# jayleicn/ClipBERT

Measured on NVIDIA H100. Metric: clips/sec fwd+bwd MSRVTT ret (ResNet50+BERT-base), higher is better.
Workload: dtype bf16

## Files before the change

### clipbert_b200/csrc/common.cuh

```cuda
#pragma once
#include <cuda.h>
#include <cuda_bf16.h>
#include <cuda_runtime.h>
#include <stdint.h>

#include "drop_cfg.h"

namespace cb {

#ifndef CB_SPIN_LIMIT
#define CB_SPIN_LIMIT (1u << 24)
#endif

__device__ __forceinline__ uint32_t smem_u32(const void* p) {
  return static_cast<uint32_t>(__cvta_generic_to_shared(p));
}

__device__ __forceinline__ void pdl_wait() { asm volatile("griddepcontrol.wait;" ::: "memory"); }
__device__ __forceinline__ void pdl_trigger() { asm volatile("griddepcontrol.launch_dependents;" ::: "memory"); }

__device__ __forceinline__ void mbar_init(uint64_t* bar, uint32_t count) {
  asm volatile("mbarrier.init.shared::cta.b64 [%0], %1;" ::"r"(smem_u32(bar)), "r"(count));
}
__device__ __forceinline__ void fence_mbar_init() {
  asm volatile("fence.mbarrier_init.release.cluster;" ::: "memory");
}
__device__ __forceinline__ void fence_proxy_async_smem() {
  asm volatile("fence.proxy.async.shared::cta;" ::: "memory");
}
__device__ __forceinline__ void mbar_expect_tx(uint64_t* bar, uint32_t bytes) {
  asm volatile("mbarrier.arrive.expect_tx.shared::cta.b64 _, [%0], %1;" ::"r"(smem_u32(bar)),
               "r"(bytes)
               : "memory");
}
__device__ __forceinline__ void mbar_arrive(uint64_t* bar) {
  asm volatile("mbarrier.arrive.shared::cta.b64 _, [%0];" ::"r"(smem_u32(bar)) : "memory");
}
__device__ __forceinline__ bool mbar_try_wait(uint64_t* bar, uint32_t parity) {
  uint32_t ok;
  asm volatile(
      "{\n\t.reg .pred p;\n\t"
      "mbarrier.try_wait.parity.shared::cta.b64 p, [%1], %2, %3;\n\t"
      "selp.u32 %0, 1, 0, p;\n\t}"
      : "=r"(ok)
      : "r"(smem_u32(bar)), "r"(parity), "r"(2000u)
      : "memory");
  return ok != 0;
}
__device__ __forceinline__ void mbar_wait(uint64_t* bar, uint32_t parity) {
  uint32_t spins = 0;
  while (!mbar_try_wait(bar, parity)) {
    if (++spins > CB_SPIN_LIMIT) __trap();
  }
}

__device__ __forceinline__ void tma_prefetch_desc(const CUtensorMap* map) {
  asm volatile("prefetch.tensormap [%0];" ::"l"(map) : "memory");
}
__device__ __forceinline__ void tma_load_2d(void* smem_dst, const CUtensorMap* map, uint64_t* bar,
                                            int c0, int c1) {
  asm volatile(
      "cp.async.bulk.tensor.2d.shared::cluster.global.mbarrier::complete_tx::bytes "
      "[%0], [%1, {%3, %4}], [%2];" ::"r"(smem_u32(smem_dst)),
      "l"(map), "r"(smem_u32(bar)), "r"(c0), "r"(c1)
      : "memory");
}

__device__ __forceinline__ void bulk_load_1d(uint32_t smem_dst, const void* gsrc, uint32_t bytes, uint64_t* bar) {
  asm volatile("cp.async.bulk.shared::cluster.global.mbarrier::complete_tx::bytes [%0], [%1], %2, [%3];" ::"r"(smem_dst), "l"(gsrc),
               "r"(bytes), "r"(smem_u32(bar))
               : "memory");
}

__device__ __forceinline__ void tma_load_2d_s32(uint32_t smem_dst, const CUtensorMap* map, uint64_t* bar, int c0, int c1) {
  asm volatile(
      "cp.async.bulk.tensor.2d.shared::cluster.global.mbarrier::complete_tx::bytes "
      "[%0], [%1, {%3, %4}], [%2];" ::"r"(smem_dst),
      "l"(map), "r"(smem_u32(bar)), "r"(c0), "r"(c1)
      : "memory");
}

__device__ __forceinline__ void tma_load_3d(void* smem_dst, const CUtensorMap* map, uint64_t* bar, int c0, int c1, int c2) {
  asm volatile(
      "cp.async.bulk.tensor.3d.shared::cluster.global.mbarrier::complete_tx::bytes "
      "[%0], [%1, {%3, %4, %5}], [%2];" ::"r"(smem_u32(smem_dst)),
      "l"(map), "r"(smem_u32(bar)), "r"(c0), "r"(c1), "r"(c2)
      : "memory");
}

__device__ __forceinline__ void tma_store_2d(const CUtensorMap* map, const void* smem_src, int c0, int c1) {
  asm volatile("cp.async.bulk.tensor.2d.global.shared::cta.bulk_group [%0, {%2, %3}], [%1];" ::"l"(map),
               "r"(smem_u32(smem_src)), "r"(c0), "r"(c1)
               : "memory");
}
__device__ __forceinline__ void tma_store_2d_s32(const CUtensorMap* map, uint32_t smem_src, int c0, int c1) {
  asm volatile("cp.async.bulk.tensor.2d.global.shared::cta.bulk_group [%0, {%2, %3}], [%1];" ::"l"(map), "r"(smem_src), "r"(c0), "r"(c1)
               : "memory");
}
__device__ __forceinline__ uint4 lds128(uint32_t saddr) {
  uint4 v;
  asm volatile("ld.shared.v4.u32 {%0, %1, %2, %3}, [%4];" : "=r"(v.x), "=r"(v.y), "=r"(v.z), "=r"(v.w) : "r"(saddr));
  return v;
}
__device__ __forceinline__ void sts128(uint32_t saddr, uint4 v) {
  asm volatile("st.shared.v4.u32 [%0], {%1, %2, %3, %4};" ::"r"(saddr), "r"(v.x), "r"(v.y), "r"(v.z), "r"(v.w) : "memory");
}
__device__ __forceinline__ void tma_store_commit() { asm volatile("cp.async.bulk.commit_group;" ::: "memory"); }
template <int N>
__device__ __forceinline__ void tma_store_wait_read() {
  asm volatile("cp.async.bulk.wait_group.read %0;" ::"n"(N) : "memory");
}
template <int N>
__device__ __forceinline__ void tma_store_wait_all() {
  asm volatile("cp.async.bulk.wait_group %0;" ::"n"(N) : "memory");
}
__device__ __forceinline__ void named_bar_sync(uint32_t id, uint32_t nthreads) {
  asm volatile("bar.sync %0, %1;" ::"r"(id), "r"(nthreads) : "memory");
}

__device__ __forceinline__ void wgmma_fence() { asm volatile("wgmma.fence.sync.aligned;" ::: "memory"); }
__device__ __forceinline__ void wgmma_commit() { asm volatile("wgmma.commit_group.sync.aligned;" ::: "memory"); }
template <int N>
__device__ __forceinline__ void wgmma_wait() {
  asm volatile("wgmma.wait_group.sync.aligned %0;" ::"n"(N) : "memory");
}
template <int R>
__device__ __forceinline__ void wgmma_fence_acc(float (&d)[R]) {
#pragma unroll
  for (int i = 0; i < R; ++i) asm volatile("" : "+f"(d[i])::"memory");
}

__device__ __forceinline__ uint64_t gmma_desc(uint32_t smem_addr, uint32_t lbo, uint32_t sbo) {
  uint64_t d = 0;
  d |= static_cast<uint64_t>((smem_addr & 0x3FFFFu) >> 4);
  d |= static_cast<uint64_t>((lbo >> 4) & 0x3FFFu) << 16;
  d |= static_cast<uint64_t>((sbo >> 4) & 0x3FFFu) << 32;
  d |= 1ull << 62;
  return d;
}

template <int TA, int TB>
__device__ __forceinline__ void wgmma_bf16_n64(float (&d)[32], uint64_t adesc, uint64_t bdesc, uint32_t accumulate) {
  asm volatile(
      "{\n\t.reg .pred p;\n\t"
      "setp.ne.b32 p, %34, 0;\n\t"
      "wgmma.mma_async.sync.aligned.m64n64k16.f32.bf16.bf16 "
      "{"
      "%0, %1, %2, %3, %4, %5, %6, %7, %8, %9, %10, %11, %12, %13, %14, %15, "
      "%16, %17, %18, %19, %20, %21, %22, %23, %24, %25, %26, %27, %28, %29, %30, %31"
      "}, %32, %33, p, 1, 1, %35, %36;\n\t}"
      : "+f"(d[0]), "+f"(d[1]), "+f"(d[2]), "+f"(d[3]), "+f"(d[4]), "+f"(d[5]), "+f"(d[6]), "+f"(d[7]),
        "+f"(d[8]), "+f"(d[9]), "+f"(d[10]), "+f"(d[11]), "+f"(d[12]), "+f"(d[13]), "+f"(d[14]), "+f"(d[15]),
        "+f"(d[16]), "+f"(d[17]), "+f"(d[18]), "+f"(d[19]), "+f"(d[20]), "+f"(d[21]), "+f"(d[22]), "+f"(d[23]),
        "+f"(d[24]), "+f"(d[25]), "+f"(d[26]), "+f"(d[27]), "+f"(d[28]), "+f"(d[29]), "+f"(d[30]), "+f"(d[31])
      : "l"(adesc), "l"(bdesc), "r"(accumulate), "n"(TA), "n"(TB));
}
template <int TA, int TB>
__device__ __forceinline__ void wgmma_bf16_n128(float (&d)[64], uint64_t adesc, uint64_t bdesc, uint32_t accumulate) {
  asm volatile(
      "{\n\t.reg .pred p;\n\t"
      "setp.ne.b32 p, %66, 0;\n\t"
      "wgmma.mma_async.sync.aligned.m64n128k16.f32.bf16.bf16 "
      "{"
      "%0, %1, %2, %3, %4, %5, %6, %7, %8, %9, %10, %11, %12, %13, %14, %15, "
      "%16, %17, %18, %19, %20, %21, %22, %23, %24, %25, %26, %27, %28, %29, %30, %31, "
      "%32, %33, %34, %35, %36, %37, %38, %39, %40, %41, %42, %43, %44, %45, %46, %47, "
      "%48, %49, %50, %51, %52, %53, %54, %55, %56, %57, %58, %59, %60, %61, %62, %63"
      "}, %64, %65, p, 1, 1, %67, %68;\n\t}"
      : "+f"(d[0]), "+f"(d[1]), "+f"(d[2]), "+f"(d[3]), "+f"(d[4]), "+f"(d[5]), "+f"(d[6]), "+f"(d[7]),
        "+f"(d[8]), "+f"(d[9]), "+f"(d[10]), "+f"(d[11]), "+f"(d[12]), "+f"(d[13]), "+f"(d[14]), "+f"(d[15]),
        "+f"(d[16]), "+f"(d[17]), "+f"(d[18]), "+f"(d[19]), "+f"(d[20]), "+f"(d[21]), "+f"(d[22]), "+f"(d[23]),
        "+f"(d[24]), "+f"(d[25]), "+f"(d[26]), "+f"(d[27]), "+f"(d[28]), "+f"(d[29]), "+f"(d[30]), "+f"(d[31]),
        "+f"(d[32]), "+f"(d[33]), "+f"(d[34]), "+f"(d[35]), "+f"(d[36]), "+f"(d[37]), "+f"(d[38]), "+f"(d[39]),
        "+f"(d[40]), "+f"(d[41]), "+f"(d[42]), "+f"(d[43]), "+f"(d[44]), "+f"(d[45]), "+f"(d[46]), "+f"(d[47]),
        "+f"(d[48]), "+f"(d[49]), "+f"(d[50]), "+f"(d[51]), "+f"(d[52]), "+f"(d[53]), "+f"(d[54]), "+f"(d[55]),
        "+f"(d[56]), "+f"(d[57]), "+f"(d[58]), "+f"(d[59]), "+f"(d[60]), "+f"(d[61]), "+f"(d[62]), "+f"(d[63])
      : "l"(adesc), "l"(bdesc), "r"(accumulate), "n"(TA), "n"(TB));
}
template <int TA, int TB>
__device__ __forceinline__ void wgmma_bf16_n256(float (&d)[128], uint64_t adesc, uint64_t bdesc, uint32_t accumulate) {
  asm volatile(
      "{\n\t.reg .pred p;\n\t"
      "setp.ne.b32 p, %130, 0;\n\t"
      "wgmma.mma_async.sync.aligned.m64n256k16.f32.bf16.bf16 "
      "{"
      "%0, %1, %2, %3, %4, %5, %6, %7, %8, %9, %10, %11, %12, %13, %14, %15, "
      "%16, %17, %18, %19, %20, %21, %22, %23, %24, %25, %26, %27, %28, %29, %30, %31, "
      "%32, %33, %34, %35, %36, %37, %38, %39, %40, %41, %42, %43, %44, %45, %46, %47, "
      "%48, %49, %50, %51, %52, %53, %54, %55, %56, %57, %58, %59, %60, %61, %62, %63, "
      "%64, %65, %66, %67, %68, %69, %70, %71, %72, %73, %74, %75, %76, %77, %78, %79, "
      "%80, %81, %82, %83, %84, %85, %86, %87, %88, %89, %90, %91, %92, %93, %94, %95, "
      "%96, %97, %98, %99, %100, %101, %102, %103, %104, %105, %106, %107, %108, %109, %110, %111, "
      "%112, %113, %114, %115, %116, %117, %118, %119, %120, %121, %122, %123, %124, %125, %126, %127"
      "}, %128, %129, p, 1, 1, %131, %132;\n\t}"
      : "+f"(d[0]), "+f"(d[1]), "+f"(d[2]), "+f"(d[3]), "+f"(d[4]), "+f"(d[5]), "+f"(d[6]), "+f"(d[7]),
        "+f"(d[8]), "+f"(d[9]), "+f"(d[10]), "+f"(d[11]), "+f"(d[12]), "+f"(d[13]), "+f"(d[14]), "+f"(d[15]),
        "+f"(d[16]), "+f"(d[17]), "+f"(d[18]), "+f"(d[19]), "+f"(d[20]), "+f"(d[21]), "+f"(d[22]), "+f"(d[23]),
        "+f"(d[24]), "+f"(d[25]), "+f"(d[26]), "+f"(d[27]), "+f"(d[28]), "+f"(d[29]), "+f"(d[30]), "+f"(d[31]),
        "+f"(d[32]), "+f"(d[33]), "+f"(d[34]), "+f"(d[35]), "+f"(d[36]), "+f"(d[37]), "+f"(d[38]), "+f"(d[39]),
        "+f"(d[40]), "+f"(d[41]), "+f"(d[42]), "+f"(d[43]), "+f"(d[44]), "+f"(d[45]), "+f"(d[46]), "+f"(d[47]),
        "+f"(d[48]), "+f"(d[49]), "+f"(d[50]), "+f"(d[51]), "+f"(d[52]), "+f"(d[53]), "+f"(d[54]), "+f"(d[55]),
        "+f"(d[56]), "+f"(d[57]), "+f"(d[58]), "+f"(d[59]), "+f"(d[60]), "+f"(d[61]), "+f"(d[62]), "+f"(d[63]),
        "+f"(d[64]), "+f"(d[65]), "+f"(d[66]), "+f"(d[67]), "+f"(d[68]), "+f"(d[69]), "+f"(d[70]), "+f"(d[71]),
        "+f"(d[72]), "+f"(d[73]), "+f"(d[74]), "+f"(d[75]), "+f"(d[76]), "+f"(d[77]), "+f"(d[78]), "+f"(d[79]),
        "+f"(d[80]), "+f"(d[81]), "+f"(d[82]), "+f"(d[83]), "+f"(d[84]), "+f"(d[85]), "+f"(d[86]), "+f"(d[87]),
        "+f"(d[88]), "+f"(d[89]), "+f"(d[90]), "+f"(d[91]), "+f"(d[92]), "+f"(d[93]), "+f"(d[94]), "+f"(d[95]),
        "+f"(d[96]), "+f"(d[97]), "+f"(d[98]), "+f"(d[99]), "+f"(d[100]), "+f"(d[101]), "+f"(d[102]), "+f"(d[103]),
        "+f"(d[104]), "+f"(d[105]), "+f"(d[106]), "+f"(d[107]), "+f"(d[108]), "+f"(d[109]), "+f"(d[110]), "+f"(d[111]),
        "+f"(d[112]), "+f"(d[113]), "+f"(d[114]), "+f"(d[115]), "+f"(d[116]), "+f"(d[117]), "+f"(d[118]), "+f"(d[119]),
        "+f"(d[120]), "+f"(d[121]), "+f"(d[122]), "+f"(d[123]), "+f"(d[124]), "+f"(d[125]), "+f"(d[126]), "+f"(d[127])
      : "l"(adesc), "l"(bdesc), "r"(accumulate), "n"(TA), "n"(TB));
}

template <int N, int TA, int TB>
__device__ __forceinline__ void wgmma_bf16(float (&d)[N / 2], uint64_t adesc, uint64_t bdesc, uint32_t accumulate) {
  if constexpr (N == 64) wgmma_bf16_n64<TA, TB>(d, adesc, bdesc, accumulate);
  else if constexpr (N == 128) wgmma_bf16_n128<TA, TB>(d, adesc, bdesc, accumulate);
  else wgmma_bf16_n256<TA, TB>(d, adesc, bdesc, accumulate);
}

__device__ __forceinline__ float warp_sum(float v) {
#pragma unroll
  for (int o = 16; o > 0; o >>= 1) v += __shfl_xor_sync(0xffffffffu, v, o);
  return v;
}
__device__ __forceinline__ float warp_max(float v) {
#pragma unroll
  for (int o = 16; o > 0; o >>= 1) v = fmaxf(v, __shfl_xor_sync(0xffffffffu, v, o));
  return v;
}

__device__ __forceinline__ void red_add_f32x4(float* addr, float4 v) {
  asm volatile("red.global.add.v4.f32 [%0], {%1, %2, %3, %4};" ::"l"(addr), "f"(v.x), "f"(v.y), "f"(v.z),
               "f"(v.w)
               : "memory");
}

__device__ __forceinline__ void red_add_f32x2(float* addr, float x, float y) {
  asm volatile("red.global.add.v2.f32 [%0], {%1, %2};" ::"l"(addr), "f"(x), "f"(y) : "memory");
}

__device__ __forceinline__ float fast_rcp(float x) {
  float r;
  asm("rcp.approx.ftz.f32 %0, %1;" : "=f"(r) : "f"(x));
  return r;
}

__device__ __forceinline__ float fast_erf(float x) {
  const float ax = fabsf(x);
  const float t = fast_rcp(fmaf(0.3275911f, ax, 1.0f));
  float p = fmaf(1.061405429f, t, -1.453152027f);
  p = fmaf(p, t, 1.421413741f);
  p = fmaf(p, t, -0.284496736f);
  p = fmaf(p, t, 0.254829592f);
  const float r = 1.0f - p * t * __expf(-ax * ax);
  return copysignf(r, x);
}
__device__ __forceinline__ float gelu_erf(float x) {
  return 0.5f * x * (1.0f + fast_erf(x * 0.70710678118654752f));
}
__device__ __forceinline__ void gelu_erf_and_grad(float x, float& y, float& g) {
  const float az = fabsf(x) * 0.70710678118654752f;
  const float t = fast_rcp(fmaf(0.3275911f, az, 1.0f));
  float p = fmaf(1.061405429f, t, -1.453152027f);
  p = fmaf(p, t, 1.421413741f);
  p = fmaf(p, t, -0.284496736f);
  p = fmaf(p, t, 0.254829592f);
  const float e = __expf(-az * az);
  const float cdf = 0.5f * (1.0f + copysignf(1.0f - p * t * e, x));
  y = x * cdf;
  g = fmaf(x * 0.3989422804014327f, e, cdf);
}
__device__ __forceinline__ float gelu_erf_grad(float x) {
  const float cdf = 0.5f * (1.0f + fast_erf(x * 0.70710678118654752f));
  const float pdf = 0.3989422804014327f * __expf(-0.5f * x * x);
  return cdf + x * pdf;
}

__device__ __forceinline__ uint64_t drop_seed(uint64_t seed, const uint64_t* offset) {
  return offset ? seed + __ldg(reinterpret_cast<const unsigned long long*>(offset)) * 0xD1342543DE82EF95ull : seed;
}
__device__ __forceinline__ DropCfg drop_resolve(DropCfg dc) {
  if (dc.thresh) dc.seed = drop_seed(dc.seed, dc.offset);
  dc.offset = nullptr;
  return dc;
}
__device__ __forceinline__ uint64_t drop_hash(uint64_t seed, uint64_t group) {
  uint64_t z = group * 0x9E3779B97F4A7C15ull + seed;
  z = (z ^ (z >> 30)) * 0xBF58476D1CE4E5B9ull;
  z = (z ^ (z >> 27)) * 0x94D049BB133111EBull;
  return z ^ (z >> 31);
}
__device__ __forceinline__ float drop_lane(uint64_t h, int lane, uint32_t thresh, float inv_keep) {
  return (static_cast<uint32_t>(h >> (16 * lane)) & 0xFFFFu) >= thresh ? inv_keep : 0.0f;
}
__device__ __forceinline__ float dropout_mult(uint64_t seed, uint64_t idx, uint32_t thresh, float inv_keep) {
  return drop_lane(drop_hash(seed, idx >> 2), static_cast<int>(idx & 3), thresh, inv_keep);
}
__device__ __forceinline__ void dropout_mult4(uint64_t seed, uint64_t idx, uint32_t thresh, float inv_keep, float (&m)[4]) {
  const uint64_t h = drop_hash(seed, idx >> 2);
#pragma unroll
  for (int j = 0; j < 4; ++j) m[j] = drop_lane(h, j, thresh, inv_keep);
}
__device__ __forceinline__ void dropout_mult2(uint64_t seed, uint64_t idx, uint32_t thresh, float inv_keep, float& m0, float& m1) {
  const uint64_t h0 = drop_hash(seed, idx >> 2);
  const int l0 = static_cast<int>(idx & 3);
  m0 = drop_lane(h0, l0, thresh, inv_keep);
  m1 = l0 == 3 ? drop_lane(drop_hash(seed, (idx >> 2) + 1), 0, thresh, inv_keep) : drop_lane(h0, l0 + 1, thresh, inv_keep);
}

__device__ __forceinline__ uint32_t pack_bf16x2(float lo, float hi) {
  __nv_bfloat162 h = __floats2bfloat162_rn(lo, hi);
  return *reinterpret_cast<uint32_t*>(&h);
}
__device__ __forceinline__ float2 unpack_bf16x2(uint32_t u) {
  __nv_bfloat162 h = *reinterpret_cast<__nv_bfloat162*>(&u);
  return __bfloat1622float2(h);
}

}
```

### clipbert_b200/csrc/gemm.cu

```cuda
#include "common.cuh"
#include "host_util.h"

namespace cb {

constexpr int BM = 128;
constexpr int BK = 64;
constexpr int CONSUMER_WARPS = 8;
constexpr int GEMM_THREADS = (CONSUMER_WARPS + 1) * 32;
constexpr int MAX_STAGES = 8;
constexpr int SMEM_LIMIT = 232448;
constexpr int SMEM_LIMIT_OCC2 = 113 * 1024;
constexpr int STG_PITCH = 36;
constexpr int STG_WARP_FLOATS = 16 * STG_PITCH;
constexpr int EPI_BYTES = CONSUMER_WARPS * STG_WARP_FLOATS * 4;
constexpr int IN_BOX_BYTES = BM * 64 * 2;
constexpr int MAX_IN_BUFS = 2;

struct GemmEpi {
  const float* scale;
  const float* shift;
  const __nv_bfloat16* residual;
  const __nv_bfloat16* aux;
  int aux_mode;
  int act;
  void* out;
  int64_t out_ld;
  int out_fp32;
  __nv_bfloat16* out2;
  int64_t out2_ld;
  int rowmap, H, W;
  uint32_t drop_thresh;
  float drop_inv_keep;
  uint64_t seed;
  const uint64_t* seed_off;
  int mn3d;
  long long* dbg;
};

__device__ __forceinline__ void dbg_stamp(const GemmEpi& epi, int slot) {
  if (epi.dbg) {
    epi.dbg[blockIdx.x * 32 + slot] = clock64();
    if (slot == 0 || slot == 11) {
      unsigned long long ns;
      asm volatile("mov.u64 %0, %%globaltimer;" : "=l"(ns));
      epi.dbg[blockIdx.x * 32 + (slot == 0 ? 12 : 13)] = static_cast<long long>(ns);
    }
  }
}

template <int BN>
struct GemmCfg {
  static constexpr int A_BYTES = BM * BK * 2;
  static constexpr int B_BYTES = BN * BK * 2;
  static constexpr int STAGE_BYTES = A_BYTES + B_BYTES;
  static constexpr int BAR_BYTES = 256;
};

enum { EK_GENERIC = 0, EK_SHIFT_ACT = 1, EK_RELU_MASK = 2, EK_DROP_RES = 3, EK_GELU_STASH = 4, EK_AUX_MUL = 5 };

template <int NC>
__device__ __forceinline__ void add_shift(float (&f)[NC], const float (&shv)[NC]) {
#pragma unroll
  for (int j = 0; j < NC; ++j) f[j] += shv[j];
}
template <int NC>
__device__ __forceinline__ void add_residual(float (&f)[NC], const uint32_t (&res16)[NC / 2]) {
#pragma unroll
  for (int j = 0; j < NC / 2; ++j) {
    const float2 r2 = unpack_bf16x2(res16[j]);
    f[2 * j] += r2.x;
    f[2 * j + 1] += r2.y;
  }
}
template <int NC>
__device__ __forceinline__ void epilogue_shift_act(float (&f)[NC], const float (&shv)[NC], bool has_shift, const uint32_t (&res16)[NC / 2], bool has_res,
                                                   bool relu) {
  if (has_shift) add_shift<NC>(f, shv);
  if (has_res) add_residual<NC>(f, res16);
  if (relu) {
#pragma unroll
    for (int j = 0; j < NC; ++j) f[j] = fmaxf(f[j], 0.0f);
  }
}
template <int NC>
__device__ __forceinline__ void epilogue_relu_mask(float (&f)[NC], const uint32_t (&res16)[NC / 2], bool has_res, const uint32_t (&aux16)[NC / 2]) {
  if (has_res) add_residual<NC>(f, res16);
#pragma unroll
  for (int j = 0; j < NC / 2; ++j) {
    const uint32_t a = aux16[j];
    f[2 * j] = ((a & 0x8000u) == 0u && (a & 0x7fffu) != 0u) ? f[2 * j] : 0.0f;
    f[2 * j + 1] = ((a & 0x80000000u) == 0u && (a & 0x7fff0000u) != 0u) ? f[2 * j + 1] : 0.0f;
  }
}
template <int NC>
__device__ __forceinline__ void epilogue_drop_res(float (&f)[NC], const float (&shv)[NC], bool has_shift, const uint32_t (&res16)[NC / 2], bool has_res,
                                                  uint64_t dseed, uint64_t didx, uint32_t thresh, float inv_keep) {
  if (has_shift) add_shift<NC>(f, shv);
#pragma unroll
  for (int j = 0; j < NC; j += 4) {
    float m[4];
    dropout_mult4(dseed, didx + j, thresh, inv_keep, m);
    f[j] *= m[0]; f[j + 1] *= m[1]; f[j + 2] *= m[2]; f[j + 3] *= m[3];
  }
  if (has_res) add_residual<NC>(f, res16);
}
template <int NC>
__device__ __forceinline__ void epilogue_gelu_stash(float (&f)[NC], const float (&shv)[NC], bool has_shift, uint32_t (&o2_16)[NC / 2]) {
  if (has_shift) add_shift<NC>(f, shv);
#pragma unroll
  for (int j = 0; j < NC / 2; ++j) {
    float y0, g0, y1, g1;
    gelu_erf_and_grad(f[2 * j], y0, g0);
    gelu_erf_and_grad(f[2 * j + 1], y1, g1);
    f[2 * j] = y0;
    f[2 * j + 1] = y1;
    o2_16[j] = pack_bf16x2(g0, g1);
  }
}
template <int NC>
__device__ __forceinline__ void epilogue_aux_mul(float (&f)[NC], const uint32_t (&res16)[NC / 2], bool has_res, const uint32_t (&aux16)[NC / 2]) {
  if (has_res) add_residual<NC>(f, res16);
#pragma unroll
  for (int j = 0; j < NC / 2; ++j) {
    const float2 a2 = unpack_bf16x2(aux16[j]);
    f[2 * j] *= a2.x;
    f[2 * j + 1] *= a2.y;
  }
}
template <int NC, bool GUARD>
__device__ __forceinline__ void epilogue_math(float (&f)[NC], const GemmEpi& epi, const float (&shv)[NC], bool has_shift, uint64_t dseed, int nb, int N,
                                              int64_t orow, const uint32_t (&res16)[NC / 2], bool has_res, const uint32_t (&aux16)[NC / 2], bool has_aux,
                                              uint32_t (&o2_16)[NC / 2], bool has_out2) {
  if (GUARD && nb >= N) return;
  if (epi.scale) {
#pragma unroll
    for (int j = 0; j < NC; j += 4) {
      if (!GUARD || nb + j + 4 <= N) {
        const float4 s4 = __ldg(reinterpret_cast<const float4*>(epi.scale + nb + j));
        f[j] *= s4.x; f[j + 1] *= s4.y; f[j + 2] *= s4.z; f[j + 3] *= s4.w;
      }
    }
  }
  if (has_shift) add_shift<NC>(f, shv);
  if (epi.drop_thresh) {
    const uint64_t base = static_cast<uint64_t>(orow) * static_cast<uint64_t>(N) + nb;
#pragma unroll
    for (int j = 0; j < NC; j += 4) {
      float m[4];
      dropout_mult4(dseed, base + j, epi.drop_thresh, epi.drop_inv_keep, m);
      f[j] *= m[0]; f[j + 1] *= m[1]; f[j + 2] *= m[2]; f[j + 3] *= m[3];
    }
  }
  if (has_res) add_residual<NC>(f, res16);
  if (epi.act == CB_ACT_GELU_STASH_GRAD) {
#pragma unroll
    for (int j = 0; j < NC / 2; ++j) {
      float y0, g0, y1, g1;
      gelu_erf_and_grad(f[2 * j], y0, g0);
      gelu_erf_and_grad(f[2 * j + 1], y1, g1);
      f[2 * j] = y0;
      f[2 * j + 1] = y1;
      if (has_out2) o2_16[j] = pack_bf16x2(g0, g1);
    }
  } else if (has_out2) {
#pragma unroll
    for (int j = 0; j < NC / 2; ++j) o2_16[j] = pack_bf16x2(f[2 * j], f[2 * j + 1]);
  }
  switch (epi.act) {
    case CB_ACT_RELU:
#pragma unroll
      for (int j = 0; j < NC; ++j) f[j] = fmaxf(f[j], 0.0f);
      break;
    case CB_ACT_GELU:
#pragma unroll
      for (int j = 0; j < NC; ++j) f[j] = gelu_erf(f[j]);
      break;
    case CB_ACT_TANH:
#pragma unroll
      for (int j = 0; j < NC; ++j) f[j] = tanhf(f[j]);
      break;
    default: break;
  }
  if (has_aux) {
    switch (epi.aux_mode) {
      case CB_AUX_RELU_MASK:
#pragma unroll
        for (int j = 0; j < NC / 2; ++j) {
          const float2 a2 = unpack_bf16x2(aux16[j]);
          f[2 * j] = a2.x > 0.0f ? f[2 * j] : 0.0f;
          f[2 * j + 1] = a2.y > 0.0f ? f[2 * j + 1] : 0.0f;
        }
        break;
      case CB_AUX_GELU_GRAD:
#pragma unroll
        for (int j = 0; j < NC / 2; ++j) {
          const float2 a2 = unpack_bf16x2(aux16[j]);
          f[2 * j] *= gelu_erf_grad(a2.x);
          f[2 * j + 1] *= gelu_erf_grad(a2.y);
        }
        break;
      case CB_AUX_TANH_GRAD:
#pragma unroll
        for (int j = 0; j < NC / 2; ++j) {
          const float2 a2 = unpack_bf16x2(aux16[j]);
          f[2 * j] *= (1.0f - a2.x * a2.x);
          f[2 * j + 1] *= (1.0f - a2.y * a2.y);
        }
        break;
      case CB_AUX_MUL:
#pragma unroll
        for (int j = 0; j < NC / 2; ++j) {
          const float2 a2 = unpack_bf16x2(aux16[j]);
          f[2 * j] *= a2.x;
          f[2 * j + 1] *= a2.y;
        }
        break;
      default: break;
    }
  }
}

struct TileInfo {
  int m0, n0, nb0, tap, it_begin, n_iters;
};

template <int BN, int MODE>
__device__ __forceinline__ TileInfo decode_tile(int tile, int tiles_m, int tiles_n, int K, int ntaps, int iters_per_split) {
  TileInfo t;
  const int nt = tile % tiles_n;
  int r = tile / tiles_n;
  const int mt = r % tiles_m;
  r /= tiles_m;
  t.m0 = mt * BM;
  t.n0 = nt * BN;
  t.nb0 = t.n0;
  const int kc = (K + BK - 1) / BK;
  if (MODE == 1) {
    t.tap = r % ntaps;
    const int split = r / ntaps;
    t.it_begin = split * iters_per_split;
    t.n_iters = min(kc, t.it_begin + iters_per_split) - t.it_begin;
  } else {
    t.tap = 0;
    t.it_begin = 0;
    t.n_iters = ntaps * kc;
  }
  return t;
}

template <int BN, int TA, int TB>
__device__ __forceinline__ void mma_tile(float (&acc)[BN / 2], uint32_t smem0, int stage_bytes, int KCH, int STAGES, int n_iters, int wg,
                                         int lane, int& s, uint32_t& ph, uint64_t* full_bar, uint64_t* empty_bar) {
  using Cfg = GemmCfg<BN>;
  int prev = -1;
  for (int i = 0; i < n_iters; i += KCH) {
    const int nch = min(KCH, n_iters - i);
    mbar_wait(&full_bar[s], ph);
    __syncwarp();
    wgmma_fence();
    wgmma_fence_acc(acc);
    for (int ch = 0; ch < nch; ++ch) {
      const uint32_t a_addr = smem0 + s * stage_bytes + ch * Cfg::STAGE_BYTES + wg * (64 * 128);
      const uint32_t b_addr = smem0 + s * stage_bytes + ch * Cfg::STAGE_BYTES + Cfg::A_BYTES;
#pragma unroll
      for (int k = 0; k < BK / 16; ++k) {
        const uint64_t ad = TA ? gmma_desc(a_addr + k * 2048, BK * 128, 1024) : gmma_desc(a_addr + k * 32, 16, 1024);
        const uint64_t bd = TB ? gmma_desc(b_addr + k * 2048, BK * 128, 1024) : gmma_desc(b_addr + k * 32, 16, 1024);
        wgmma_bf16<BN, TA, TB>(acc, ad, bd, (i > 0 || ch > 0 || k > 0) ? 1u : 0u);
      }
    }
    wgmma_commit();
    wgmma_wait<1>();
    wgmma_fence_acc(acc);
    if (prev >= 0) {
      __syncwarp();
      if (lane == 0) mbar_arrive(&empty_bar[prev]);
    }
    prev = s;
    if (++s == STAGES) { s = 0; ph ^= 1; }
  }
  wgmma_wait<0>();
  wgmma_fence_acc(acc);
  if (prev >= 0) {
    __syncwarp();
    if (lane == 0) mbar_arrive(&empty_bar[prev]);
  }
}

template <int BN>
__device__ __forceinline__ void wgrad_epilogue(const float (&acc)[BN / 2], float* obase, int64_t out_ld, const float* scale, int M, int N, int r0,
                                               int n0, int lane) {
  const int r1 = r0 + 8;
  const float rs0 = (r0 < M && scale) ? scale[r0] : 1.0f;
  const float rs1 = (r1 < M && scale) ? scale[r1] : 1.0f;
#pragma unroll
  for (int j = 0; j < BN / 8; ++j) {
    const int n = n0 + j * 8 + 2 * (lane & 3);
    if (n < N) {
      if (r0 < M) red_add_f32x2(obase + static_cast<int64_t>(r0) * out_ld + n, acc[4 * j] * rs0, acc[4 * j + 1] * rs0);
      if (r1 < M) red_add_f32x2(obase + static_cast<int64_t>(r1) * out_ld + n, acc[4 * j + 2] * rs1, acc[4 * j + 3] * rs1);
    }
  }
}

__device__ __forceinline__ uint32_t swz128(uint32_t box, int r, int q) { return box + r * 128 + ((q ^ (r & 7)) << 4); }

template <int BN, int MODE, int OCC>
__global__ void __launch_bounds__(GEMM_THREADS, OCC)
    gemm_kernel(const __grid_constant__ CUtensorMap tmA, const __grid_constant__ CUtensorMap tmB, const __grid_constant__ CUtensorMap tmR,
                const __grid_constant__ CUtensorMap tmX, int M, int N, int K, int ntaps, int tap_w, int tap_sign, int iters_per_split,
                int tiles_m, int tiles_n, int total_tiles, int STAGES, int KCH, int N_IN, int epi_bytes, GemmEpi epi) {
  using Cfg = GemmCfg<BN>;
  extern __shared__ uint8_t smem_raw[];
  uint8_t* smem = reinterpret_cast<uint8_t*>((reinterpret_cast<uintptr_t>(smem_raw) + 1023) & ~static_cast<uintptr_t>(1023));
  const int stage_bytes = KCH * Cfg::STAGE_BYTES;
  const bool has_res = MODE != 1 && epi.residual != nullptr, has_aux = MODE != 1 && epi.aux != nullptr;
  constexpr int IN_TILE_BYTES = (BN / 64) * IN_BOX_BYTES;
  const int in_bytes = (has_res + has_aux) * IN_TILE_BYTES;
  uint8_t* in_base = smem + STAGES * stage_bytes;
  uint8_t* stg_base = in_base + N_IN * in_bytes;
  uint64_t* full_bar = reinterpret_cast<uint64_t*>(stg_base + epi_bytes);
  uint64_t* empty_bar = full_bar + MAX_STAGES;
  uint64_t* in_full = empty_bar + MAX_STAGES;
  uint64_t* in_empty = in_full + MAX_IN_BUFS;

  const int warp = threadIdx.x >> 5;
  const int lane = threadIdx.x & 31;
  const int unit = blockIdx.x;
  const int n_units = gridDim.x;
  if (threadIdx.x == 0) dbg_stamp(epi, 0);
  pdl_trigger();
  if (threadIdx.x == 0) {
    tma_prefetch_desc(&tmA);
    tma_prefetch_desc(&tmB);
    if (has_res) tma_prefetch_desc(&tmR);
    if (has_aux) tma_prefetch_desc(&tmX);
    for (int s = 0; s < STAGES; ++s) {
      mbar_init(&full_bar[s], 1);
      mbar_init(&empty_bar[s], CONSUMER_WARPS);
    }
    for (int b = 0; b < N_IN; ++b) {
      mbar_init(&in_full[b], 1);
      mbar_init(&in_empty[b], CONSUMER_WARPS);
    }
    fence_mbar_init();
  }
  __syncthreads();
  const int kc_per_tap = (K + BK - 1) / BK;
  pdl_wait();
  if (threadIdx.x == 0) dbg_stamp(epi, 1);

  if (warp >= CONSUMER_WARPS) {
    if (warp == CONSUMER_WARPS && lane == 0) {
      constexpr int A_BOXES = (MODE == 1) ? BM / 64 : 1;
      constexpr int B_BOXES = (MODE == 0) ? 1 : BN / 64;
      int s = 0;
      uint32_t ph = 0;
      int ib = 0;
      uint32_t iph = 0;
      auto load_inputs = [&](const TileInfo& t) {
        uint64_t* bar;
        uint8_t* dst;
        if (N_IN) {
          mbar_wait(&in_empty[ib], iph ^ 1);
          bar = &in_full[ib];
          dst = in_base + ib * in_bytes;
          if (++ib == N_IN) { ib = 0; iph ^= 1; }
        } else {
          mbar_wait(&empty_bar[s], ph ^ 1);
          bar = &full_bar[s];
          dst = smem + s * stage_bytes;
          if (++s == STAGES) { s = 0; ph ^= 1; }
        }
        mbar_expect_tx(bar, in_bytes);
        if (has_res) {
#pragma unroll
          for (int j = 0; j < BN / 64; ++j) tma_load_2d(dst + j * IN_BOX_BYTES, &tmR, bar, t.n0 + j * 64, t.m0);
          dst += IN_TILE_BYTES;
        }
        if (has_aux) {
#pragma unroll
          for (int j = 0; j < BN / 64; ++j) tma_load_2d(dst + j * IN_BOX_BYTES, &tmX, bar, t.n0 + j * 64, t.m0);
        }
      };
      for (int tile = unit; tile < total_tiles; tile += n_units) {
        const TileInfo t = decode_tile<BN, MODE>(tile, tiles_m, tiles_n, K, ntaps, iters_per_split);
        const bool inputs_first = tile < unit + N_IN * n_units;
        if (in_bytes && inputs_first) load_inputs(t);
        for (int i = 0; i < t.n_iters; i += KCH) {
          const int nch = min(KCH, t.n_iters - i);
          mbar_wait(&empty_bar[s], ph ^ 1);
          mbar_expect_tx(&full_bar[s], nch * Cfg::STAGE_BYTES);
          auto load = [&](void* dst, const CUtensorMap* map, int c0, int c1) { tma_load_2d(dst, map, &full_bar[s], c0, c1); };
          int kit = t.it_begin + i;
          int tp = 0, kc = kit;
          if (MODE != 1 && ntaps > 1) { tp = kit / kc_per_tap; kc = kit - tp * kc_per_tap; }
          for (int ch = 0; ch < nch; ++ch, ++kit) {
            uint8_t* sa = smem + s * stage_bytes + ch * Cfg::STAGE_BYTES;
            uint8_t* sb = sa + Cfg::A_BYTES;
            if (MODE == 1) {
              int shift = 0;
              if (ntaps == 9) shift = tap_sign * ((t.tap / 3 - 1) * tap_w + (t.tap % 3 - 1));
              const int p = kit * BK;
              if (epi.mn3d) {
                tma_load_3d(sa, &tmA, &full_bar[s], 0, p, t.m0 >> 6);
                tma_load_3d(sb, &tmB, &full_bar[s], 0, p + shift, t.nb0 >> 6);
              } else {
#pragma unroll
                for (int j = 0; j < A_BOXES; ++j) load(sa + j * (BK * 128), &tmA, t.m0 + j * 64, p);
#pragma unroll
                for (int j = 0; j < B_BOXES; ++j) load(sb + j * (BK * 128), &tmB, t.nb0 + j * 64, p + shift);
              }
            } else {
              int shift = 0;
              if (ntaps == 9) shift = tap_sign * ((tp / 3 - 1) * tap_w + (tp % 3 - 1));
              else if (ntaps > 1) shift = tap_sign * tp * tap_w;
              load(sa, &tmA, kc * BK, t.m0 + shift);
              if (MODE == 0) {
                load(sb, &tmB, tp * K + kc * BK, t.nb0);
              } else if (epi.mn3d) {
                tma_load_3d(sb, &tmB, &full_bar[s], 0, kc * BK, (tp * N + t.nb0) >> 6);
              } else {
#pragma unroll
                for (int j = 0; j < B_BOXES; ++j) load(sb + j * (BK * 128), &tmB, tp * N + t.nb0 + j * 64, kc * BK);
              }
              if (++kc == kc_per_tap) { kc = 0; ++tp; }
            }
          }
          if (++s == STAGES) { s = 0; ph ^= 1; }
          if (i == 0 && tile == unit) dbg_stamp(epi, 2);
        }
        if (in_bytes && !inputs_first) load_inputs(t);
      }
      dbg_stamp(epi, 3);
    }
    return;
  }

  const int wg = warp >> 2;
  const int wrow = wg * 64 + (warp & 3) * 16;
  const uint32_t smem0 = smem_u32(smem);
  const uint64_t dseed = epi.drop_thresh ? drop_seed(epi.seed, epi.seed_off) : 0ull;
  float acc[BN / 2];
  int s = 0;
  uint32_t ph = 0;
  int local = 0;

  const int er = lane & 15, eh = lane >> 4;
  float* stg = reinterpret_cast<float*>(stg_base) + warp * STG_WARP_FLOATS;
  const bool has_out2 = epi.out2 != nullptr;
  const bool has_shift = epi.shift != nullptr;
  const bool full = (N & 15) == 0 && epi.scale == nullptr;
  const bool drop = epi.drop_thresh != 0;
  int kind = EK_GENERIC;
  if (full) {
    if (!drop && !has_out2 && !has_aux && (epi.act == CB_ACT_NONE || epi.act == CB_ACT_RELU)) kind = EK_SHIFT_ACT;
    else if (!drop && !has_out2 && !has_shift && has_aux && epi.aux_mode == CB_AUX_RELU_MASK && epi.act == CB_ACT_NONE) kind = EK_RELU_MASK;
    else if (drop && !has_out2 && !has_aux && epi.act == CB_ACT_NONE) kind = EK_DROP_RES;
    else if (!drop && has_out2 && !has_aux && !has_res && epi.act == CB_ACT_GELU_STASH_GRAD) kind = EK_GELU_STASH;
    else if (!drop && !has_out2 && !has_shift && has_aux && epi.aux_mode == CB_AUX_MUL && epi.act == CB_ACT_NONE) kind = EK_AUX_MUL;
  }
  const bool kind_relu = epi.act == CB_ACT_RELU;
  const bool guard = (N & 15) != 0;

  for (int tile = unit; tile < total_tiles; tile += n_units, ++local) {
    const TileInfo t = decode_tile<BN, MODE>(tile, tiles_m, tiles_n, K, ntaps, iters_per_split);
    if (local == 0 && warp == 0 && lane == 0) dbg_stamp(epi, 4);
    mma_tile<BN, MODE == 1, MODE != 0>(acc, smem0, stage_bytes, KCH, STAGES, t.n_iters, wg, lane, s, ph, full_bar, empty_bar);
    if (local == 0 && warp == 0 && lane == 0) dbg_stamp(epi, 5);

    if (MODE == 1) {
      wgrad_epilogue<BN>(acc, reinterpret_cast<float*>(epi.out) + static_cast<int64_t>(t.tap) * N, epi.out_ld, epi.scale, M, N,
                         t.m0 + wrow + (lane >> 2), t.n0, lane);
      continue;
    }

    const int m = t.m0 + wrow + er;
    bool row_ok = m < M;
    int64_t orow = m;
    if (epi.rowmap == CB_ROWMAP_PAD) {
      const int hw = epi.H * epi.W;
      const int img = m / hw;
      const int r = m - img * hw;
      const int y = r / epi.W, x = r - y * epi.W;
      orow = (static_cast<int64_t>(img) * (epi.H + 2) + y + 1) * (epi.W + 2) + x + 1;
    } else if (epi.rowmap == CB_ROWMAP_UNPAD) {
      const int wp = epi.W + 2, hp = epi.H + 2;
      const int img = m / (hp * wp);
      const int r = m - img * (hp * wp);
      const int y = r / wp, x = r - y * wp;
      row_ok = row_ok && y >= 1 && y <= epi.H && x >= 1 && x <= epi.W;
      orow = (static_cast<int64_t>(img) * epi.H + (y - 1)) * epi.W + (x - 1);
    }
    const int ib = N_IN == 2 ? (local & 1) : 0;
    const uint32_t in_buf = N_IN ? smem_u32(in_base) + ib * in_bytes : smem0 + s * stage_bytes;
    if (in_bytes) {
      if (N_IN) mbar_wait(&in_full[ib], static_cast<uint32_t>(N_IN == 2 ? local >> 1 : local) & 1u);
      else mbar_wait(&full_bar[s], ph);
    }
#pragma unroll
    for (int sc = 0; sc < BN / 32; ++sc) {
      __syncwarp();
#pragma unroll
      for (int jj = 0; jj < 4; ++jj) {
        const int j = sc * 4 + jj;
        float* p = stg + (lane >> 2) * STG_PITCH + jj * 8 + 2 * (lane & 3);
        *reinterpret_cast<float2*>(p) = make_float2(acc[4 * j], acc[4 * j + 1]);
        *reinterpret_cast<float2*>(p + 8 * STG_PITCH) = make_float2(acc[4 * j + 2], acc[4 * j + 3]);
      }
      __syncwarp();
      const int nb = t.n0 + sc * 32 + eh * 16;
      if (!row_ok || nb >= N) continue;
      constexpr int NC = 16;
      float f[NC];
      const uint32_t srow = smem_u32(stg + er * STG_PITCH + eh * 16);
#pragma unroll
      for (int j = 0; j < NC / 4; ++j) {
        const uint4 u = lds128(srow + j * 16);
        f[4 * j] = __uint_as_float(u.x); f[4 * j + 1] = __uint_as_float(u.y);
        f[4 * j + 2] = __uint_as_float(u.z); f[4 * j + 3] = __uint_as_float(u.w);
      }
      uint32_t res16[NC / 2], aux16[NC / 2];
      const int tc = sc * 32 + eh * 16;
      const int q = (tc & 63) >> 3;
      if (has_res) {
#pragma unroll
        for (int j = 0; j < 2; ++j) {
          const uint4 u = lds128(swz128(in_buf + (tc >> 6) * IN_BOX_BYTES, wrow + er, q + j));
          res16[4 * j] = u.x; res16[4 * j + 1] = u.y; res16[4 * j + 2] = u.z; res16[4 * j + 3] = u.w;
        }
      }
      if (has_aux) {
#pragma unroll
        for (int j = 0; j < 2; ++j) {
          const uint4 u = lds128(swz128(in_buf + (has_res ? IN_TILE_BYTES : 0) + (tc >> 6) * IN_BOX_BYTES, wrow + er, q + j));
          aux16[4 * j] = u.x; aux16[4 * j + 1] = u.y; aux16[4 * j + 2] = u.z; aux16[4 * j + 3] = u.w;
        }
      }
      float shv[NC];
      if (has_shift) {
#pragma unroll
        for (int j = 0; j < NC; j += 4) {
          float4 s4 = make_float4(0.f, 0.f, 0.f, 0.f);
          if (nb + j + 4 <= N) s4 = __ldg(reinterpret_cast<const float4*>(epi.shift + nb + j));
          shv[j] = s4.x; shv[j + 1] = s4.y; shv[j + 2] = s4.z; shv[j + 3] = s4.w;
        }
      }
      uint32_t o2_16[NC / 2];
      switch (kind) {
        case EK_SHIFT_ACT: epilogue_shift_act<NC>(f, shv, has_shift, res16, has_res, kind_relu); break;
        case EK_RELU_MASK: epilogue_relu_mask<NC>(f, res16, has_res, aux16); break;
        case EK_DROP_RES:
          epilogue_drop_res<NC>(f, shv, has_shift, res16, has_res, dseed, static_cast<uint64_t>(orow) * static_cast<uint64_t>(N) + nb, epi.drop_thresh,
                                epi.drop_inv_keep);
          break;
        case EK_GELU_STASH: epilogue_gelu_stash<NC>(f, shv, has_shift, o2_16); break;
        case EK_AUX_MUL: epilogue_aux_mul<NC>(f, res16, has_res, aux16); break;
        default:
          if (guard) epilogue_math<NC, true>(f, epi, shv, has_shift, dseed, nb, N, orow, res16, has_res, aux16, has_aux, o2_16, has_out2);
          else epilogue_math<NC, false>(f, epi, shv, has_shift, dseed, nb, N, orow, res16, has_res, aux16, has_aux, o2_16, has_out2);
      }
      if (epi.out_fp32) {
        float* o = reinterpret_cast<float*>(epi.out) + orow * epi.out_ld + nb;
#pragma unroll
        for (int j = 0; j < NC; j += 4)
          if (nb + j + 4 <= N) *reinterpret_cast<float4*>(o + j) = make_float4(f[j], f[j + 1], f[j + 2], f[j + 3]);
      } else {
        __nv_bfloat16* o = reinterpret_cast<__nv_bfloat16*>(epi.out) + orow * epi.out_ld + nb;
#pragma unroll
        for (int j = 0; j < 2; ++j)
          if (nb + 8 * j + 8 <= N)
            *reinterpret_cast<uint4*>(o + 8 * j) = make_uint4(pack_bf16x2(f[8 * j], f[8 * j + 1]), pack_bf16x2(f[8 * j + 2], f[8 * j + 3]),
                                                              pack_bf16x2(f[8 * j + 4], f[8 * j + 5]), pack_bf16x2(f[8 * j + 6], f[8 * j + 7]));
      }
      if (has_out2) {
        __nv_bfloat16* o = epi.out2 + orow * epi.out2_ld + nb;
#pragma unroll
        for (int j = 0; j < 2; ++j)
          if (nb + 8 * j + 8 <= N) *reinterpret_cast<uint4*>(o + 8 * j) = make_uint4(o2_16[4 * j], o2_16[4 * j + 1], o2_16[4 * j + 2], o2_16[4 * j + 3]);
      }
    }
    if (in_bytes) {
      __syncwarp();
      if (lane == 0) mbar_arrive(N_IN ? &in_empty[ib] : &empty_bar[s]);
      if (!N_IN && ++s == STAGES) { s = 0; ph ^= 1; }
    }
    if (local == 0 && warp == 0 && lane == 0) dbg_stamp(epi, 8);
  }
  if (threadIdx.x == 0) dbg_stamp(epi, 11);
}

static int g_sm_limit = 0;
static int sm_count() {
  static int n = 0;
  if (n == 0) {
    int dev = 0;
    cudaGetDevice(&dev);
    cudaDeviceGetAttribute(&n, cudaDevAttrMultiProcessorCount, dev);
    if (n <= 0) n = 132;
  }
  return (g_sm_limit > 0 && g_sm_limit < n) ? g_sm_limit : n;
}

static long long* g_gemm_timeline = nullptr;
static int g_force_kch = 0;
static int g_mn3d = 1;

struct SmemPlan {
  int epi_bytes, kch, stages, chunk_bytes, n_in;
};
static SmemPlan plan_ring(int bn, bool staging, int kiters, int force_kch, int occ, int in_bytes, int n_in) {
  SmemPlan p;
  const int limit = occ == 2 ? SMEM_LIMIT_OCC2 : SMEM_LIMIT;
  p.chunk_bytes = BM * BK * 2 + bn * BK * 2;
  p.epi_bytes = staging ? EPI_BYTES : 0;
  p.n_in = n_in;
  const int chunks_fit = (limit - 1024 - GemmCfg<64>::BAR_BYTES - p.epi_bytes - n_in * in_bytes) / p.chunk_bytes;
  p.kch = 1;
  if (force_kch > 0) p.kch = force_kch;
  else if (g_force_kch > 0) p.kch = g_force_kch;
  else if (kiters >= 4 && chunks_fit >= 8) p.kch = 4;
  else if (kiters >= 2 && chunks_fit >= 4) p.kch = 2;
  if (p.kch > kiters) p.kch = kiters;
  if (p.kch > 1 && chunks_fit / p.kch < 2) p.kch = 1;
  p.stages = chunks_fit / p.kch;
  if (p.stages > MAX_STAGES) p.stages = MAX_STAGES;
  const int stage_iters = ceil_div(kiters, p.kch);
  if (p.stages > stage_iters + 1) p.stages = stage_iters + 1 > 2 ? stage_iters + 1 : 2;
  return p;
}
static SmemPlan plan_smem(int bn, bool staging, int kiters, int force_kch = 0, int occ = 1, int in_bytes = 0) {
  const SmemPlan none = plan_ring(bn, staging, kiters, force_kch, occ, 0, 0);
  if (in_bytes == 0) return none;
  const SmemPlan two = plan_ring(bn, staging, kiters, force_kch, occ, in_bytes, 2);
  if (two.stages >= 2 && two.stages * two.kch >= kiters) return two;
  if (kiters > 4 && none.stages >= 2 && none.kch * none.chunk_bytes >= in_bytes) return none;
  return plan_ring(bn, staging, kiters, force_kch, occ, in_bytes, 1);
}
static int epi_in_bytes(const cb_gemm_desc& d, int bn) {
  return d.mode == CB_GEMM_WGRAD ? 0 : ((d.residual != nullptr) + (d.aux != nullptr)) * (bn / 64) * IN_BOX_BYTES;
}

template <int BN, int MODE, int OCC = 1>
static int launch_gemm(const cb_gemm_desc& d, const GemmEpi& epi_in, cudaStream_t stream) {
  GemmEpi epi = epi_in;
  using Cfg = GemmCfg<BN>;
  constexpr int LIMIT = OCC == 2 ? SMEM_LIMIT_OCC2 : SMEM_LIMIT;
  static bool attr_set = false;
  auto kern = gemm_kernel<BN, MODE, OCC>;
  if (!attr_set) {
    cudaError_t e = cudaFuncSetAttribute(kern, cudaFuncAttributeMaxDynamicSharedMemorySize, LIMIT);
    if (e == cudaSuccess && OCC == 2)
      e = cudaFuncSetAttribute(kern, cudaFuncAttributePreferredSharedMemoryCarveout, cudaSharedmemCarveoutMaxShared);
    if (e != cudaSuccess) {
      set_error("cudaFuncSetAttribute(smem=%d): %s", LIMIT, cudaGetErrorString(e));
      return CB_ERR_CUDA;
    }
    attr_set = true;
  }
  alignas(64) CUtensorMap ta, tb, tr, tx;
  bool mn3d = false;
  int iters_per_split = 0;
  const int tiles_m = ceil_div(d.m, BM), tiles_n = ceil_div(d.n, BN);
  int total = tiles_m * tiles_n;
  int kiters;
  bool ok;
  if (MODE == 0) {
    ok = get_tmap_2d(&ta, d.a, d.k, d.a_rows, d.a_ld, BK, BM) &&
         get_tmap_2d(&tb, d.b, static_cast<uint64_t>(d.k) * d.ntaps, d.b_rows, d.b_ld, BK, BN);
    kiters = ceil_div(d.k, BK) * d.ntaps;
  } else if (MODE == 2) {
    ok = get_tmap_2d(&ta, d.a, d.k, d.a_rows, d.a_ld, BK, BM);
    mn3d = g_mn3d && d.n % 64 == 0 &&
           get_tmap_3d_mn(&tb, d.b, static_cast<uint64_t>(d.n) * d.ntaps, d.b_rows, d.b_ld, BK, BN / 64);
    if (!mn3d) ok = ok && get_tmap_2d(&tb, d.b, static_cast<uint64_t>(d.n) * d.ntaps, d.b_rows, d.b_ld, 64, BK);
    kiters = ceil_div(d.k, BK) * d.ntaps;
  } else {
    mn3d = g_mn3d && d.m % 64 == 0 && d.n % 64 == 0 && get_tmap_3d_mn(&ta, d.a, d.m, d.a_rows, d.a_ld, BK, BM / 64) &&
           get_tmap_3d_mn(&tb, d.b, d.n, d.b_rows, d.b_ld, BK, BN / 64);
    ok = mn3d || (get_tmap_2d(&ta, d.a, d.m, d.a_rows, d.a_ld, 64, BK) && get_tmap_2d(&tb, d.b, d.n, d.b_rows, d.b_ld, 64, BK));
    const int kc = ceil_div(d.k, BK);
    int splits = d.split_k < 1 ? 1 : d.split_k;
    if (splits > kc) splits = kc;
    iters_per_split = ceil_div(kc, splits);
    splits = ceil_div(kc, iters_per_split);
    total *= splits * d.ntaps;
    kiters = iters_per_split;
  }
  tr = ta;
  tx = ta;
  if (MODE != 1 && d.residual) ok = ok && get_tmap_2d(&tr, d.residual, d.n, d.m, d.res_ld, 64, BM);
  if (MODE != 1 && d.aux) ok = ok && get_tmap_2d(&tx, d.aux, d.n, d.m, d.aux_ld, 64, BM);
  if (!ok) return CB_ERR_CUDA;
  epi.mn3d = mn3d ? 1 : 0;
  const int units = sm_count() * OCC;
  const int grid = total < units ? total : units;
  const int in_bytes = epi_in_bytes(d, BN);
  const SmemPlan sp = plan_smem(BN, MODE != 1, kiters, (d.reserved >> 8) & 15, OCC, in_bytes);
  const int epi_bytes = sp.epi_bytes, kch = sp.kch, stages = sp.stages;
  if (stages < 2) {
    set_error("cb_gemm: not enough shared memory for a 2-stage pipeline (BN=%d, epilogue %d B + inputs %d B, %d CTA(s) per SM)", BN, epi_bytes,
              in_bytes, OCC);
    return CB_ERR_INVALID;
  }
  const int smem_bytes = stages * kch * Cfg::STAGE_BYTES + sp.n_in * in_bytes + epi_bytes + Cfg::BAR_BYTES + 1024;
  launch_gemm_k(kern, grid, GEMM_THREADS, smem_bytes, stream, ta, tb, tr, tx, d.m, d.n, d.k, d.ntaps, d.tap_w, d.tap_sign, iters_per_split,
                tiles_m, tiles_n, total, stages, kch, sp.n_in, epi_bytes, epi);
  return check_launch("cb_gemm");
}

struct LaunchCfg {
  int bn, splits;
};

static int g_occ2_mode = 1;
static double g_occ2_max_gflop = 0.0;

static LaunchCfg choose_config(const cb_gemm_desc& d, int occ = 1) {
  const int units = sm_count() * occ;
  const int kc = ceil_div(d.k, BK);
  const bool wgrad = d.mode == CB_GEMM_WGRAD;
  static const int cand[3] = {64, 128, 256};
  LaunchCfg best = {0, 1};
  double best_cost = 1e30;
  for (int c = 0; c < 3; ++c) {
    const int bn = cand[c];
    if (occ == 2 && bn > 64) continue;
    if (d.block_n && bn != d.block_n) continue;
    if (!d.block_n && !wgrad && bn == 256) continue;
    if (bn > 64 && d.n <= bn / 2) continue;
    const int64_t base = static_cast<int64_t>(ceil_div(d.m, BM)) * ceil_div(d.n, bn) * (wgrad ? d.ntaps : 1);
    const int max_split = wgrad ? (d.split_k > 0 ? d.split_k : (kc < 32 ? kc : 32)) : 1;
    for (int sp = (wgrad && d.split_k > 0) ? d.split_k : 1; sp <= max_split; ++sp) {
      const int ips = ceil_div(wgrad ? kc : kc * d.ntaps, sp);
      const int real_sp = wgrad ? ceil_div(kc, ips) : 1;
      const int64_t tiles = base * real_sp;
      const double rounds = static_cast<double>((tiles + units - 1) / units);
      const SmemPlan pl = plan_smem(bn, !wgrad, ips, (d.reserved >> 8) & 15, occ, epi_in_bytes(d, bn));
      if (pl.stages < 2) continue;
      const double shallow = (pl.stages * pl.kch < 3 && ips > 2) ? 3.0 : 1.0;
      const double stage_cost = 450.0 + pl.kch * pl.chunk_bytes / (60.0 / occ);
      const double epi = wgrad ? bn * 24.0 : bn * 30.0;
      const double cost = rounds * (ceil_div(ips, pl.kch) * stage_cost * shallow + epi) + 2500.0;
      if (cost < best_cost) {
        best_cost = cost;
        best = {bn, real_sp};
      }
    }
  }
  if (best.bn == 0 && occ == 1) best = {64, 1};
  return best;
}

constexpr int WG_MAX_PROBLEMS = 8;
struct WgradProblem {
  CUtensorMap tmA, tmB;
  float* out;
  const float* scale;
  int64_t out_ld;
  int M, N, K;
  int ntaps, tap_w, tap_sign;
  int iters_per_split, tiles_m, tiles_n;
  int tile_begin;
  int mn3d;
};
struct WgradGroup {
  int nprob, total_tiles;
  WgradProblem p[WG_MAX_PROBLEMS];
};
struct WgTile {
  int pi, m0, n0, tap, it_begin, n_iters;
};
__device__ __forceinline__ WgTile wg_decode(const WgradGroup& g, int tile) {
  WgTile t;
  int pi = 0;
  while (pi + 1 < g.nprob && tile >= g.p[pi + 1].tile_begin) ++pi;
  const WgradProblem& P = g.p[pi];
  int r = tile - P.tile_begin;
  const int nt = r % P.tiles_n;
  r /= P.tiles_n;
  const int mt = r % P.tiles_m;
  r /= P.tiles_m;
  t.pi = pi;
  t.m0 = mt * BM;
  t.tap = r % P.ntaps;
  const int split = r / P.ntaps;
  const int kc = (P.K + BK - 1) / BK;
  t.it_begin = split * P.iters_per_split;
  t.n_iters = min(kc, t.it_begin + P.iters_per_split) - t.it_begin;
  t.n0 = nt;
  return t;
}

template <int BN>
__global__ void __launch_bounds__(GEMM_THREADS, 1)
    wgrad_group_kernel(const __grid_constant__ WgradGroup g, int STAGES, int KCH) {
  using Cfg = GemmCfg<BN>;
  extern __shared__ uint8_t smem_raw[];
  uint8_t* smem = reinterpret_cast<uint8_t*>((reinterpret_cast<uintptr_t>(smem_raw) + 1023) & ~static_cast<uintptr_t>(1023));
  const int stage_bytes = KCH * Cfg::STAGE_BYTES;
  uint64_t* full_bar = reinterpret_cast<uint64_t*>(smem + STAGES * stage_bytes);
  uint64_t* empty_bar = full_bar + MAX_STAGES;
  const int warp = threadIdx.x >> 5, lane = threadIdx.x & 31;
  const int unit = blockIdx.x, n_units = gridDim.x;
  pdl_trigger();
  if (threadIdx.x == 0) {
    for (int i = 0; i < g.nprob; ++i) {
      tma_prefetch_desc(&g.p[i].tmA);
      tma_prefetch_desc(&g.p[i].tmB);
    }
    for (int s = 0; s < STAGES; ++s) {
      mbar_init(&full_bar[s], 1);
      mbar_init(&empty_bar[s], CONSUMER_WARPS);
    }
    fence_mbar_init();
  }
  __syncthreads();
  pdl_wait();

  if (warp >= CONSUMER_WARPS) {
    if (warp == CONSUMER_WARPS && lane == 0) {
      int s = 0;
      uint32_t ph = 0;
      for (int tile = unit; tile < g.total_tiles; tile += n_units) {
        const WgTile t = wg_decode(g, tile);
        const WgradProblem& P = g.p[t.pi];
        const int n0 = t.n0 * BN;
        int shift = 0;
        if (P.ntaps == 9) shift = P.tap_sign * ((t.tap / 3 - 1) * P.tap_w + (t.tap % 3 - 1));
        for (int i = 0; i < t.n_iters; i += KCH) {
          const int nch = min(KCH, t.n_iters - i);
          mbar_wait(&empty_bar[s], ph ^ 1);
          mbar_expect_tx(&full_bar[s], nch * Cfg::STAGE_BYTES);
          int kit = t.it_begin + i;
          for (int ch = 0; ch < nch; ++ch, ++kit) {
            uint8_t* sa = smem + s * stage_bytes + ch * Cfg::STAGE_BYTES;
            uint8_t* sb = sa + Cfg::A_BYTES;
            const int p = kit * BK;
            if (P.mn3d) {
              tma_load_3d(sa, &P.tmA, &full_bar[s], 0, p, t.m0 >> 6);
              tma_load_3d(sb, &P.tmB, &full_bar[s], 0, p + shift, n0 >> 6);
            } else {
#pragma unroll
              for (int j = 0; j < BM / 64; ++j) tma_load_2d(sa + j * (BK * 128), &P.tmA, &full_bar[s], t.m0 + j * 64, p);
#pragma unroll
              for (int j = 0; j < BN / 64; ++j) tma_load_2d(sb + j * (BK * 128), &P.tmB, &full_bar[s], n0 + j * 64, p + shift);
            }
          }
          if (++s == STAGES) { s = 0; ph ^= 1; }
        }
      }
    }
    return;
  }

  const int wg = warp >> 2;
  const int wrow = wg * 64 + (warp & 3) * 16;
  const uint32_t smem0 = smem_u32(smem);
  float acc[BN / 2];
  int s = 0;
  uint32_t ph = 0;
  for (int tile = unit; tile < g.total_tiles; tile += n_units) {
    const WgTile t = wg_decode(g, tile);
    const WgradProblem& P = g.p[t.pi];
    mma_tile<BN, 1, 1>(acc, smem0, stage_bytes, KCH, STAGES, t.n_iters, wg, lane, s, ph, full_bar, empty_bar);
    wgrad_epilogue<BN>(acc, P.out + static_cast<int64_t>(t.tap) * P.N, P.out_ld, P.scale, P.M, P.N, t.m0 + wrow + (lane >> 2), t.n0 * BN, lane);
  }
}

template <int BN>
static int launch_wgrad_group(const cb_gemm_desc* descs, int n, int splits, cudaStream_t stream) {
  using Cfg = GemmCfg<BN>;
  static bool attr_set = false;
  auto kern = wgrad_group_kernel<BN>;
  if (!attr_set) {
    cudaError_t e = cudaFuncSetAttribute(kern, cudaFuncAttributeMaxDynamicSharedMemorySize, SMEM_LIMIT);
    if (e != cudaSuccess) {
      set_error("cudaFuncSetAttribute(smem=%d): %s", SMEM_LIMIT, cudaGetErrorString(e));
      return CB_ERR_CUDA;
    }
    attr_set = true;
  }
  alignas(64) WgradGroup g;
  g.nprob = n;
  int total = 0, max_iters = 0;
  for (int i = 0; i < n; ++i) {
    const cb_gemm_desc& d = descs[i];
    WgradProblem& P = g.p[i];
    const bool mn3d = g_mn3d && d.m % 64 == 0 && d.n % 64 == 0 && get_tmap_3d_mn(&P.tmA, d.a, d.m, d.a_rows, d.a_ld, BK, BM / 64) &&
                      get_tmap_3d_mn(&P.tmB, d.b, d.n, d.b_rows, d.b_ld, BK, BN / 64);
    if (!mn3d && !(get_tmap_2d(&P.tmA, d.a, d.m, d.a_rows, d.a_ld, 64, BK) && get_tmap_2d(&P.tmB, d.b, d.n, d.b_rows, d.b_ld, 64, BK)))
      return CB_ERR_CUDA;
    P.mn3d = mn3d ? 1 : 0;
    P.out = static_cast<float*>(d.out);
    P.scale = d.scale;
    P.out_ld = d.out_ld;
    P.M = d.m; P.N = d.n; P.K = d.k;
    P.ntaps = d.ntaps; P.tap_w = d.tap_w; P.tap_sign = d.tap_sign;
    const int kc = ceil_div(d.k, BK);
    int sp = splits < 1 ? 1 : (splits > kc ? kc : splits);
    P.iters_per_split = ceil_div(kc, sp);
    sp = ceil_div(kc, P.iters_per_split);
    P.tiles_m = ceil_div(d.m, BM);
    P.tiles_n = ceil_div(d.n, BN);
    P.tile_begin = total;
    total += P.tiles_m * P.tiles_n * d.ntaps * sp;
    if (P.iters_per_split > max_iters) max_iters = P.iters_per_split;
  }
  g.total_tiles = total;
  const SmemPlan sp = plan_smem(BN, false, max_iters, 0, 1);
  if (sp.stages < 2) {
    set_error("cb_gemm_wgrad_group: not enough shared memory for a 2-stage pipeline (BN=%d)", BN);
    return CB_ERR_INVALID;
  }
  const int smem_bytes = sp.stages * sp.kch * Cfg::STAGE_BYTES + Cfg::BAR_BYTES + 1024;
  const int units = sm_count();
  launch_gemm_k(kern, total < units ? total : units, GEMM_THREADS, smem_bytes, stream, g, sp.stages, sp.kch);
  return check_launch("cb_gemm_wgrad_group");
}

}

extern "C" void cb_debug_gemm_timeline(void* device_buf) { cb::g_gemm_timeline = static_cast<long long*>(device_buf); }
extern "C" void cb_debug_gemm_kch(int kch) { cb::g_force_kch = kch; }
extern "C" void cb_debug_gemm_mn3d(int on) { cb::g_mn3d = on ? 1 : 0; }
extern "C" void cb_debug_gemm_occ2(int mode, double max_gflop) {
  cb::g_occ2_mode = mode < 0 ? 0 : (mode > 2 ? 2 : mode);
  cb::g_occ2_max_gflop = max_gflop;
}
extern "C" void cb_debug_gemm_sm_limit(int n) { cb::g_sm_limit = n > 0 ? n : 0; }

extern "C" int cb_gemm(const cb_gemm_desc* dp, void* stream_v) {
  using namespace cb;
  CB_REQUIRE(dp != nullptr, "cb_gemm: null descriptor");
  const cb_gemm_desc& d = *dp;
  cudaStream_t stream = static_cast<cudaStream_t>(stream_v);
  CB_REQUIRE(d.a && d.b && d.out, "cb_gemm: null operand pointer");
  CB_REQUIRE(d.m > 0 && d.n > 0 && d.k > 0, "cb_gemm: empty problem m=%d n=%d k=%d", d.m, d.n, d.k);
  CB_REQUIRE(d.ntaps == 1 || d.ntaps == 9 || (d.ntaps == 4 && d.mode == CB_GEMM_TN),
             "cb_gemm: ntaps must be 1, 9 (3x3 conv) or 4 (row taps, TN only) (got %d)", d.ntaps);
  CB_REQUIRE(d.mode == CB_GEMM_TN || d.mode == CB_GEMM_WGRAD || d.mode == CB_GEMM_NN, "cb_gemm: bad mode %d", d.mode);
  CB_REQUIRE(d.dropout_p >= 0.0f && d.dropout_p < 1.0f, "cb_gemm: dropout_p out of range");

  GemmEpi epi;
  epi.scale = d.scale;
  epi.shift = d.shift;
  epi.residual = static_cast<const __nv_bfloat16*>(d.residual);
  epi.aux = static_cast<const __nv_bfloat16*>(d.aux);
  epi.aux_mode = d.aux ? d.aux_mode : CB_AUX_NONE;
  epi.act = d.act;
  epi.out = d.out;
  epi.out_ld = d.out_ld;
  epi.out_fp32 = d.out_fp32;
  epi.out2 = static_cast<__nv_bfloat16*>(d.out2);
  epi.out2_ld = d.out2_ld;
  epi.rowmap = d.rowmap;
  epi.H = d.map_h;
  epi.W = d.map_w;
  epi.seed = d.dropout_seed;
  epi.dbg = g_gemm_timeline;
  epi.mn3d = 0;
  {
    const DropCfg dc = make_drop(d.dropout_p, d.dropout_seed);
    epi.drop_thresh = dc.thresh;
    epi.drop_inv_keep = dc.inv_keep;
    epi.seed_off = dc.offset;
  }
  const double gflop = 2.0e-9 * d.m * d.n * d.k * d.ntaps;
  const bool want_occ2 = (d.reserved & 64) == 0 && (!d.block_n || d.block_n == 64) &&
                         ((d.reserved & 32) ? g_occ2_mode >= 1 : (g_occ2_mode == 2 && (g_occ2_max_gflop <= 0.0 || gflop <= g_occ2_max_gflop)));

  if (d.mode == CB_GEMM_TN || d.mode == CB_GEMM_NN) {
    const bool nn = d.mode == CB_GEMM_NN;
    CB_REQUIRE(d.n % 8 == 0, "cb_gemm(TN): n must be a multiple of 8 (got %d)", d.n);
    CB_REQUIRE(d.k % 8 == 0, "cb_gemm(TN): k must be a multiple of 8 (got %d)", d.k);
    CB_REQUIRE(d.out_ld % 8 == 0, "cb_gemm(TN): out_ld must be a multiple of 8");
    CB_REQUIRE(!d.residual || d.res_ld % 8 == 0, "cb_gemm(TN): res_ld must be a multiple of 8");
    CB_REQUIRE(!d.aux || d.aux_ld % 8 == 0, "cb_gemm(TN): aux_ld must be a multiple of 8");
    CB_REQUIRE((reinterpret_cast<uintptr_t>(d.residual) & 15) == 0, "cb_gemm(TN): residual must be 16-byte aligned");
    CB_REQUIRE((reinterpret_cast<uintptr_t>(d.aux) & 15) == 0, "cb_gemm(TN): aux must be 16-byte aligned");
    CB_REQUIRE(!d.out2 || d.out2_ld % 8 == 0, "cb_gemm(TN): out2_ld must be a multiple of 8");
    CB_REQUIRE(!(d.out2 && d.out_fp32), "cb_gemm(TN): out2 requires a bf16 primary output");
    CB_REQUIRE(d.rowmap == CB_ROWMAP_NONE || (d.map_h > 0 && d.map_w > 0), "cb_gemm: rowmap needs map_h/map_w");
    CB_REQUIRE(d.ntaps == 1 || d.tap_w > 2, "cb_gemm: tap modes need tap_w (padded row pitch in pixels)");
    if (want_occ2) {
      const LaunchCfg l2 = choose_config(d, 2);
      if (l2.bn == 64) return nn ? launch_gemm<64, 2, 2>(d, epi, stream) : launch_gemm<64, 0, 2>(d, epi, stream);
    }
    const LaunchCfg lc = choose_config(d);
    switch (lc.bn) {
      case 64: return nn ? launch_gemm<64, 2>(d, epi, stream) : launch_gemm<64, 0>(d, epi, stream);
      case 128: return nn ? launch_gemm<128, 2>(d, epi, stream) : launch_gemm<128, 0>(d, epi, stream);
      case 256: return nn ? launch_gemm<256, 2>(d, epi, stream) : launch_gemm<256, 0>(d, epi, stream);
      default: CB_REQUIRE(false, "cb_gemm: block_n must be 0, 64, 128 or 256 (got %d)", lc.bn);
    }
  } else {
    CB_REQUIRE(d.out_fp32 == 1, "cb_gemm(WGRAD): output must be fp32");
    CB_REQUIRE(d.m % 8 == 0 && d.n % 8 == 0, "cb_gemm(WGRAD): m, n must be multiples of 8 (got %d, %d)", d.m, d.n);
    CB_REQUIRE(d.out_ld % 4 == 0, "cb_gemm(WGRAD): out_ld must be a multiple of 4");
    CB_REQUIRE((reinterpret_cast<uintptr_t>(d.out) & 15) == 0, "cb_gemm(WGRAD): out must be 16-byte aligned");
    if (want_occ2) {
      const LaunchCfg l2 = choose_config(d, 2);
      cb_gemm_desc d2 = d;
      d2.split_k = l2.splits;
      if (l2.bn == 64) return launch_gemm<64, 1, 2>(d2, epi, stream);
    }
    const LaunchCfg lc = choose_config(d);
    cb_gemm_desc d2 = d;
    d2.split_k = lc.splits;
    switch (lc.bn) {
      case 64: return launch_gemm<64, 1>(d2, epi, stream);
      case 128: return launch_gemm<128, 1>(d2, epi, stream);
      case 256: return launch_gemm<256, 1>(d2, epi, stream);
      default: CB_REQUIRE(false, "cb_gemm(WGRAD): block_n must be 0, 64, 128 or 256 (got %d)", lc.bn);
    }
  }
  return CB_ERR_INVALID;
}

extern "C" int cb_gemm_wgrad_group(const cb_gemm_desc* descs, int n, void* stream_v) {
  using namespace cb;
  CB_REQUIRE(descs != nullptr && n >= 1, "cb_gemm_wgrad_group: no problems");
  cudaStream_t stream = static_cast<cudaStream_t>(stream_v);
  bool groupable = n >= 2 && n <= WG_MAX_PROBLEMS;
  for (int i = 0; i < n; ++i) {
    const cb_gemm_desc& d = descs[i];
    CB_REQUIRE(d.mode == CB_GEMM_WGRAD && d.out_fp32 == 1, "cb_gemm_wgrad_group: problem %d is not an fp32 WGRAD descriptor", i);
    CB_REQUIRE(d.a && d.b && d.out && d.m > 0 && d.n > 0 && d.k > 0, "cb_gemm_wgrad_group: problem %d: null operand / empty shape", i);
    CB_REQUIRE(d.m % 8 == 0 && d.n % 8 == 0 && d.out_ld % 4 == 0 && (reinterpret_cast<uintptr_t>(d.out) & 15) == 0,
               "cb_gemm_wgrad_group: problem %d: m, n multiples of 8, out 16-byte aligned, out_ld a multiple of 4", i);
    CB_REQUIRE(d.ntaps == 1 || d.ntaps == 9, "cb_gemm_wgrad_group: problem %d: ntaps must be 1 or 9", i);
    if (d.k * 2 < descs[0].k || descs[0].k * 2 < d.k) groupable = false;
  }
  if (!groupable) {
    for (int i = 0; i < n; ++i) {
      const int rc = cb_gemm(&descs[i], stream_v);
      if (rc != CB_OK) return rc;
    }
    return CB_OK;
  }
  int min_n = descs[0].n;
  for (int i = 1; i < n; ++i) min_n = descs[i].n < min_n ? descs[i].n : min_n;
  const int bn = min_n >= 192 ? 256 : (min_n >= 96 ? 128 : 64);
  int64_t base = 0;
  int kc_min = 1 << 30;
  for (int i = 0; i < n; ++i) {
    base += static_cast<int64_t>(ceil_div(descs[i].m, BM)) * ceil_div(descs[i].n, bn) * descs[i].ntaps;
    const int kc = ceil_div(descs[i].k, BK);
    kc_min = kc < kc_min ? kc : kc_min;
  }
  const int sms = sm_count();
  int best_split = 1;
  double best_cost = 1e30;
  for (int sp = 1; sp <= 8 && sp <= kc_min; ++sp) {
    const double waves = static_cast<double>((base * sp + sms - 1) / sms);
    const double cost = waves / sp + 0.06 * sp;
    if (cost < best_cost) { best_cost = cost; best_split = sp; }
  }
  if (bn == 256) return launch_wgrad_group<256>(descs, n, best_split, stream);
  if (bn == 128) return launch_wgrad_group<128>(descs, n, best_split, stream);
  return launch_wgrad_group<64>(descs, n, best_split, stream);
}
```

Before: 2958.

## Add ping-pong warp-specialized GEMM kernel for TN/NN with register rebalancing

Splits forward/dgrad GEMMs into a new ping-pong kernel: one producer warpgroup and two consumer warpgroups that each take alternating tiles and hand off the tensor cores through named barriers. One warpgroup's epilogue can then overlap the other's main loop. Register counts are rebalanced with setmaxnreg, the tile cost model now assumes half-hidden epilogues, and the occ2 and BN=256 paths are dropped for TN/NN. Wgrad stays on the old kernel. Risks include fewer options for wide tiles, an extra pipeline stage cap for staging, and waits that no longer have a spin guard.

After: 3156 (median of 6 runs). 1.07x the previous value.

```diff
diff --git a/clipbert_b200/csrc/common.cuh b/clipbert_b200/csrc/common.cuh
--- a/clipbert_b200/csrc/common.cuh
+++ b/clipbert_b200/csrc/common.cuh
@@ -35,6 +35,11 @@
 }
 __device__ __forceinline__ void mbar_arrive(uint64_t* bar) {
   asm volatile("mbarrier.arrive.shared::cta.b64 _, [%0];" ::"r"(smem_u32(bar)) : "memory");
+}
+__device__ __forceinline__ void mbar_arrive_if(uint64_t* bar, bool pred) {
+  asm volatile("{\n\t.reg .pred p;\n\tsetp.ne.b32 p, %1, 0;\n\t@p mbarrier.arrive.shared::cta.b64 _, [%0];\n\t}" ::"r"(smem_u32(bar)),
+               "r"(static_cast<uint32_t>(pred))
+               : "memory");
 }
 __device__ __forceinline__ bool mbar_try_wait(uint64_t* bar, uint32_t parity) {
   uint32_t ok;
@@ -53,6 +58,10 @@
     if (++spins > CB_SPIN_LIMIT) __trap();
   }
 }
+__device__ __forceinline__ void mbar_wait_unguarded(uint64_t* bar, uint32_t parity) {
+  while (!mbar_try_wait(bar, parity)) {
+  }
+}
 
 __device__ __forceinline__ void tma_prefetch_desc(const CUtensorMap* map) {
   asm volatile("prefetch.tensormap [%0];" ::"l"(map) : "memory");
@@ -116,6 +125,17 @@
 }
 __device__ __forceinline__ void named_bar_sync(uint32_t id, uint32_t nthreads) {
   asm volatile("bar.sync %0, %1;" ::"r"(id), "r"(nthreads) : "memory");
+}
+__device__ __forceinline__ void named_bar_arrive(uint32_t id, uint32_t nthreads) {
+  asm volatile("bar.arrive %0, %1;" ::"r"(id), "r"(nthreads) : "memory");
+}
+template <uint32_t NREG>
+__device__ __forceinline__ void setmaxnreg_dec() {
+  asm volatile("setmaxnreg.dec.sync.aligned.u32 %0;" ::"n"(NREG));
+}
+template <uint32_t NREG>
+__device__ __forceinline__ void setmaxnreg_inc() {
+  asm volatile("setmaxnreg.inc.sync.aligned.u32 %0;" ::"n"(NREG));
 }
 
 __device__ __forceinline__ void wgmma_fence() { asm volatile("wgmma.fence.sync.aligned;" ::: "memory"); }
diff --git a/clipbert_b200/csrc/gemm.cu b/clipbert_b200/csrc/gemm.cu
--- a/clipbert_b200/csrc/gemm.cu
+++ b/clipbert_b200/csrc/gemm.cu
@@ -7,6 +7,10 @@
 constexpr int BK = 64;
 constexpr int CONSUMER_WARPS = 8;
 constexpr int GEMM_THREADS = (CONSUMER_WARPS + 1) * 32;
+constexpr int PP_THREADS = 3 * 128;
+constexpr int PP_PRODUCER_REGS = 40;
+constexpr int PP_CONSUMER_REGS = 232;
+constexpr int PP_BAR_TURN = 1;
 constexpr int MAX_STAGES = 8;
 constexpr int SMEM_LIMIT = 232448;
 constexpr int SMEM_LIMIT_OCC2 = 113 * 1024;
@@ -14,7 +18,6 @@
 constexpr int STG_WARP_FLOATS = 16 * STG_PITCH;
 constexpr int EPI_BYTES = CONSUMER_WARPS * STG_WARP_FLOATS * 4;
 constexpr int IN_BOX_BYTES = BM * 64 * 2;
-constexpr int MAX_IN_BUFS = 2;
 
 struct GemmEpi {
   const float* scale;
@@ -287,6 +290,54 @@
   }
 }
 
+template <int BN, int TB>
+__device__ __forceinline__ void mma_tile_pp(float (&acc)[2][BN / 2], uint32_t smem0, int stage_bytes, int KCH, int STAGES, int n_iters,
+                                            int lane, int& s, uint32_t& ph, uint64_t* full_bar, uint64_t* empty_bar, int pass_bar,
+                                            bool in_stage) {
+  using Cfg = GemmCfg<BN>;
+  int prev = -1;
+  for (int i = 0; i < n_iters; i += KCH) {
+    const int nch = min(KCH, n_iters - i);
+    mbar_wait_unguarded(&full_bar[s], ph);
+    __syncwarp();
+    wgmma_fence();
+    wgmma_fence_acc(acc[0]);
+    wgmma_fence_acc(acc[1]);
+    for (int ch = 0; ch < nch; ++ch) {
+      const uint32_t a_addr = smem0 + s * stage_bytes + ch * Cfg::STAGE_BYTES;
+      const uint32_t b_addr = a_addr + Cfg::A_BYTES;
+#pragma unroll
+      for (int k = 0; k < BK / 16; ++k) {
+        const uint64_t bd = TB ? gmma_desc(b_addr + k * 2048, BK * 128, 1024) : gmma_desc(b_addr + k * 32, 16, 1024);
+        const uint32_t accum = (i > 0 || ch > 0 || k > 0) ? 1u : 0u;
+#pragma unroll
+        for (int h = 0; h < 2; ++h) wgmma_bf16<BN, 0, TB>(acc[h], gmma_desc(a_addr + h * (64 * 128) + k * 32, 16, 1024), bd, accum);
+      }
+    }
+    wgmma_commit();
+    wgmma_wait<1>();
+    wgmma_fence_acc(acc[0]);
+    wgmma_fence_acc(acc[1]);
+    if (prev >= 0) {
+      __syncwarp();
+      mbar_arrive_if(&empty_bar[prev], lane == 0);
+    }
+    prev = s;
+    if (++s == STAGES) { s = 0; ph ^= 1; }
+    if (pass_bar && i + KCH >= n_iters) {
+      if (in_stage) mbar_wait_unguarded(&full_bar[s], ph);
+      named_bar_arrive(pass_bar, 2 * 128);
+    }
+  }
+  wgmma_wait<0>();
+  wgmma_fence_acc(acc[0]);
+  wgmma_fence_acc(acc[1]);
+  if (prev >= 0) {
+    __syncwarp();
+    mbar_arrive_if(&empty_bar[prev], lane == 0);
+  }
+}
+
 template <int BN>
 __device__ __forceinline__ void wgrad_epilogue(const float (&acc)[BN / 2], float* obase, int64_t out_ld, const float* scale, int M, int N, int r0,
                                                int n0, int lane) {
@@ -305,26 +356,27 @@
 
 __device__ __forceinline__ uint32_t swz128(uint32_t box, int r, int q) { return box + r * 128 + ((q ^ (r & 7)) << 4); }
 
-template <int BN, int MODE, int OCC>
-__global__ void __launch_bounds__(GEMM_THREADS, OCC)
-    gemm_kernel(const __grid_constant__ CUtensorMap tmA, const __grid_constant__ CUtensorMap tmB, const __grid_constant__ CUtensorMap tmR,
-                const __grid_constant__ CUtensorMap tmX, int M, int N, int K, int ntaps, int tap_w, int tap_sign, int iters_per_split,
-                int tiles_m, int tiles_n, int total_tiles, int STAGES, int KCH, int N_IN, int epi_bytes, GemmEpi epi) {
+template <int BN, int MODE>
+__global__ void __launch_bounds__(PP_THREADS, 1)
+    gemm_pingpong_kernel(const __grid_constant__ CUtensorMap tmA, const __grid_constant__ CUtensorMap tmB, const __grid_constant__ CUtensorMap tmR,
+                         const __grid_constant__ CUtensorMap tmX, int M, int N, int K, int ntaps, int tap_w, int tap_sign, int tiles_m,
+                         int tiles_n, int total_tiles, int STAGES, int KCH, int N_IN, GemmEpi epi) {
+  static_assert(MODE != 1 && BN <= 128, "TN / NN tiles of 128 x 64 or 128 x 128");
   using Cfg = GemmCfg<BN>;
   extern __shared__ uint8_t smem_raw[];
   uint8_t* smem = reinterpret_cast<uint8_t*>((reinterpret_cast<uintptr_t>(smem_raw) + 1023) & ~static_cast<uintptr_t>(1023));
   const int stage_bytes = KCH * Cfg::STAGE_BYTES;
-  const bool has_res = MODE != 1 && epi.residual != nullptr, has_aux = MODE != 1 && epi.aux != nullptr;
+  const bool has_res = epi.residual != nullptr, has_aux = epi.aux != nullptr;
   constexpr int IN_TILE_BYTES = (BN / 64) * IN_BOX_BYTES;
   const int in_bytes = (has_res + has_aux) * IN_TILE_BYTES;
   uint8_t* in_base = smem + STAGES * stage_bytes;
   uint8_t* stg_base = in_base + N_IN * in_bytes;
-  uint64_t* full_bar = reinterpret_cast<uint64_t*>(stg_base + epi_bytes);
+  uint64_t* full_bar = reinterpret_cast<uint64_t*>(stg_base + EPI_BYTES);
   uint64_t* empty_bar = full_bar + MAX_STAGES;
   uint64_t* in_full = empty_bar + MAX_STAGES;
-  uint64_t* in_empty = in_full + MAX_IN_BUFS;
-
-  const int warp = threadIdx.x >> 5;
+  uint64_t* in_empty = in_full + 2;
+
+  const int warp = __shfl_sync(0xffffffffu, static_cast<int>(threadIdx.x >> 5), 0);
   const int lane = threadIdx.x & 31;
   const int unit = blockIdx.x;
   const int n_units = gridDim.x;
@@ -337,35 +389,39 @@
     if (has_aux) tma_prefetch_desc(&tmX);
     for (int s = 0; s < STAGES; ++s) {
       mbar_init(&full_bar[s], 1);
-      mbar_init(&empty_bar[s], CONSUMER_WARPS);
-    }
-    for (int b = 0; b < N_IN; ++b) {
+      mbar_init(&empty_bar[s], 4);
+    }
+    for (int b = 0; b < 2; ++b) {
       mbar_init(&in_full[b], 1);
-      mbar_init(&in_empty[b], CONSUMER_WARPS);
+      mbar_init(&in_empty[b], 4);
     }
     fence_mbar_init();
   }
   __syncthreads();
   const int kc_per_tap = (K + BK - 1) / BK;
+  const int n_iters = ntaps * kc_per_tap;
+  const bool in_stage = in_bytes && !N_IN;
+  const int tile_stages = (n_iters + KCH - 1) / KCH + (in_stage ? 1 : 0);
   pdl_wait();
   if (threadIdx.x == 0) dbg_stamp(epi, 1);
 
-  if (warp >= CONSUMER_WARPS) {
-    if (warp == CONSUMER_WARPS && lane == 0) {
-      constexpr int A_BOXES = (MODE == 1) ? BM / 64 : 1;
+  if (warp < 4) {
+    setmaxnreg_dec<PP_PRODUCER_REGS>();
+    if (warp == 0 && lane == 0) {
       constexpr int B_BOXES = (MODE == 0) ? 1 : BN / 64;
       int s = 0;
       uint32_t ph = 0;
-      int ib = 0;
-      uint32_t iph = 0;
-      auto load_inputs = [&](const TileInfo& t) {
+      auto load_inputs = [&](int tile) {
+        const TileInfo t = decode_tile<BN, MODE>(tile, tiles_m, tiles_n, K, ntaps, 0);
         uint64_t* bar;
         uint8_t* dst;
         if (N_IN) {
-          mbar_wait(&in_empty[ib], iph ^ 1);
-          bar = &in_full[ib];
-          dst = in_base + ib * in_bytes;
-          if (++ib == N_IN) { ib = 0; iph ^= 1; }
+          const int local = (tile - unit) / n_units;
+          const int b = N_IN == 2 ? (local & 1) : 0;
+          const int uses = N_IN == 2 ? (local >> 1) : local;
+          mbar_wait(&in_empty[b], (static_cast<uint32_t>(uses) & 1u) ^ 1u);
+          bar = &in_full[local & 1];
+          dst = in_base + b * in_bytes;
         } else {
           mbar_wait(&empty_bar[s], ph ^ 1);
           bar = &full_bar[s];
@@ -383,71 +439,63 @@
           for (int j = 0; j < BN / 64; ++j) tma_load_2d(dst + j * IN_BOX_BYTES, &tmX, bar, t.n0 + j * 64, t.m0);
         }
       };
+      int pend = -1;
       for (int tile = unit; tile < total_tiles; tile += n_units) {
-        const TileInfo t = decode_tile<BN, MODE>(tile, tiles_m, tiles_n, K, ntaps, iters_per_split);
+        const TileInfo t = decode_tile<BN, MODE>(tile, tiles_m, tiles_n, K, ntaps, 0);
         const bool inputs_first = tile < unit + N_IN * n_units;
-        if (in_bytes && inputs_first) load_inputs(t);
-        for (int i = 0; i < t.n_iters; i += KCH) {
-          const int nch = min(KCH, t.n_iters - i);
+        if (in_bytes && N_IN && inputs_first) load_inputs(tile);
+        for (int i = 0; i < n_iters; i += KCH) {
+          const int nch = min(KCH, n_iters - i);
           mbar_wait(&empty_bar[s], ph ^ 1);
           mbar_expect_tx(&full_bar[s], nch * Cfg::STAGE_BYTES);
-          auto load = [&](void* dst, const CUtensorMap* map, int c0, int c1) { tma_load_2d(dst, map, &full_bar[s], c0, c1); };
-          int kit = t.it_begin + i;
-          int tp = 0, kc = kit;
-          if (MODE != 1 && ntaps > 1) { tp = kit / kc_per_tap; kc = kit - tp * kc_per_tap; }
-          for (int ch = 0; ch < nch; ++ch, ++kit) {
+          int tp = 0, kc = i;
+          if (ntaps > 1) { tp = i / kc_per_tap; kc = i - tp * kc_per_tap; }
+          for (int ch = 0; ch < nch; ++ch) {
             uint8_t* sa = smem + s * stage_bytes + ch * Cfg::STAGE_BYTES;
             uint8_t* sb = sa + Cfg::A_BYTES;
-            if (MODE == 1) {
-              int shift = 0;
-              if (ntaps == 9) shift = tap_sign * ((t.tap / 3 - 1) * tap_w + (t.tap % 3 - 1));
-              const int p = kit * BK;
-              if (epi.mn3d) {
-                tma_load_3d(sa, &tmA, &full_bar[s], 0, p, t.m0 >> 6);
-                tma_load_3d(sb, &tmB, &full_bar[s], 0, p + shift, t.nb0 >> 6);
-              } else {
-#pragma unroll
-                for (int j = 0; j < A_BOXES; ++j) load(sa + j * (BK * 128), &tmA, t.m0 + j * 64, p);
-#pragma unroll
-                for (int j = 0; j < B_BOXES; ++j) load(sb + j * (BK * 128), &tmB, t.nb0 + j * 64, p + shift);
-              }
+            int shift = 0;
+            if (ntaps == 9) shift = tap_sign * ((tp / 3 - 1) * tap_w + (tp % 3 - 1));
+            else if (ntaps > 1) shift = tap_sign * tp * tap_w;
+            tma_load_2d(sa, &tmA, &full_bar[s], kc * BK, t.m0 + shift);
+            if (MODE == 0) {
+              tma_load_2d(sb, &tmB, &full_bar[s], tp * K + kc * BK, t.nb0);
+            } else if (epi.mn3d) {
+              tma_load_3d(sb, &tmB, &full_bar[s], 0, kc * BK, (tp * N + t.nb0) >> 6);
             } else {
-              int shift = 0;
-              if (ntaps == 9) shift = tap_sign * ((tp / 3 - 1) * tap_w + (tp % 3 - 1));
-              else if (ntaps > 1) shift = tap_sign * tp * tap_w;
-              load(sa, &tmA, kc * BK, t.m0 + shift);
-              if (MODE == 0) {
-                load(sb, &tmB, tp * K + kc * BK, t.nb0);
-              } else if (epi.mn3d) {
-                tma_load_3d(sb, &tmB, &full_bar[s], 0, kc * BK, (tp * N + t.nb0) >> 6);
-              } else {
-#pragma unroll
-                for (int j = 0; j < B_BOXES; ++j) load(sb + j * (BK * 128), &tmB, tp * N + t.nb0 + j * 64, kc * BK);
-              }
-              if (++kc == kc_per_tap) { kc = 0; ++tp; }
+#pragma unroll
+              for (int j = 0; j < B_BOXES; ++j) tma_load_2d(sb + j * (BK * 128), &tmB, &full_bar[s], tp * N + t.nb0 + j * 64, kc * BK);
             }
+            if (++kc == kc_per_tap) { kc = 0; ++tp; }
           }
           if (++s == STAGES) { s = 0; ph ^= 1; }
           if (i == 0 && tile == unit) dbg_stamp(epi, 2);
         }
-        if (in_bytes && !inputs_first) load_inputs(t);
+        if (in_stage) load_inputs(tile);
+        if (pend >= 0) load_inputs(pend);
+        pend = (in_bytes && N_IN && !inputs_first) ? tile : -1;
       }
+      if (pend >= 0) load_inputs(pend);
       dbg_stamp(epi, 3);
     }
     return;
   }
 
-  const int wg = warp >> 2;
-  const int wrow = wg * 64 + (warp & 3) * 16;
+  setmaxnreg_inc<PP_CONSUMER_REGS>();
+  const int wg = (warp >> 2) - 1;
+  const int wq = warp & 3;
   const uint32_t smem0 = smem_u32(smem);
   const uint64_t dseed = epi.drop_thresh ? drop_seed(epi.seed, epi.seed_off) : 0ull;
-  float acc[BN / 2];
+  float acc[2][BN / 2];
   int s = 0;
   uint32_t ph = 0;
-  int local = 0;
+  auto ring_skip = [&](int n) {
+    s += n;
+    while (s >= STAGES) { s -= STAGES; ph ^= 1; }
+  };
+  if (wg == 1) ring_skip(tile_stages);
 
   const int er = lane & 15, eh = lane >> 4;
-  float* stg = reinterpret_cast<float*>(stg_base) + warp * STG_WARP_FLOATS;
+  float* stg = reinterpret_cast<float*>(stg_base) + (warp - 4) * STG_WARP_FLOATS;
   const bool has_out2 = epi.out2 != nullptr;
   const bool has_shift = epi.shift != nullptr;
   const bool full = (N & 15) == 0 && epi.scale == nullptr;
@@ -463,128 +511,218 @@
   const bool kind_relu = epi.act == CB_ACT_RELU;
   const bool guard = (N & 15) != 0;
 
-  for (int tile = unit; tile < total_tiles; tile += n_units, ++local) {
-    const TileInfo t = decode_tile<BN, MODE>(tile, tiles_m, tiles_n, K, ntaps, iters_per_split);
-    if (local == 0 && warp == 0 && lane == 0) dbg_stamp(epi, 4);
-    mma_tile<BN, MODE == 1, MODE != 0>(acc, smem0, stage_bytes, KCH, STAGES, t.n_iters, wg, lane, s, ph, full_bar, empty_bar);
-    if (local == 0 && warp == 0 && lane == 0) dbg_stamp(epi, 5);
-
-    if (MODE == 1) {
-      wgrad_epilogue<BN>(acc, reinterpret_cast<float*>(epi.out) + static_cast<int64_t>(t.tap) * N, epi.out_ld, epi.scale, M, N,
-                         t.m0 + wrow + (lane >> 2), t.n0, lane);
-      continue;
-    }
-
-    const int m = t.m0 + wrow + er;
-    bool row_ok = m < M;
-    int64_t orow = m;
-    if (epi.rowmap == CB_ROWMAP_PAD) {
-      const int hw = epi.H * epi.W;
-      const int img = m / hw;
-      const int r = m - img * hw;
-      const int y = r / epi.W, x = r - y * epi.W;
-      orow = (static_cast<int64_t>(img) * (epi.H + 2) + y + 1) * (epi.W + 2) + x + 1;
-    } else if (epi.rowmap == CB_ROWMAP_UNPAD) {
-      const int wp = epi.W + 2, hp = epi.H + 2;
-      const int img = m / (hp * wp);
-      const int r = m - img * (hp * wp);
-      const int y = r / wp, x = r - y * wp;
-      row_ok = row_ok && y >= 1 && y <= epi.H && x >= 1 && x <= epi.W;
-      orow = (static_cast<int64_t>(img) * epi.H + (y - 1)) * epi.W + (x - 1);
-    }
-    const int ib = N_IN == 2 ? (local & 1) : 0;
-    const uint32_t in_buf = N_IN ? smem_u32(in_base) + ib * in_bytes : smem0 + s * stage_bytes;
+  for (int local = wg, tile = unit + wg * n_units; tile < total_tiles; local += 2, tile += 2 * n_units) {
+    const TileInfo t = decode_tile<BN, MODE>(tile, tiles_m, tiles_n, K, ntaps, 0);
+    if (local > 0) named_bar_sync(PP_BAR_TURN + wg, 2 * 128);
+    const int pass = tile + n_units < total_tiles ? PP_BAR_TURN + (wg ^ 1) : 0;
+    mma_tile_pp<BN, MODE != 0>(acc, smem0, stage_bytes, KCH, STAGES, n_iters, lane, s, ph, full_bar, empty_bar, pass, in_stage);
+
+    const uint32_t in_buf = N_IN ? smem_u32(in_base) + (N_IN == 2 ? wg : 0) * in_bytes : smem0 + s * stage_bytes;
     if (in_bytes) {
-      if (N_IN) mbar_wait(&in_full[ib], static_cast<uint32_t>(N_IN == 2 ? local >> 1 : local) & 1u);
-      else mbar_wait(&full_bar[s], ph);
+      if (N_IN) mbar_wait_unguarded(&in_full[wg], static_cast<uint32_t>(local >> 1) & 1u);
+      else mbar_wait_unguarded(&full_bar[s], ph);
+    }
+    int orow_half[2];
+#pragma unroll
+    for (int h = 0; h < 2; ++h) {
+      const int m = t.m0 + h * 64 + wq * 16 + er;
+      bool row_ok = m < M;
+      int64_t orow = m;
+      if (epi.rowmap == CB_ROWMAP_PAD) {
+        const int hw = epi.H * epi.W;
+        const int img = m / hw;
+        const int r = m - img * hw;
+        const int y = r / epi.W, x = r - y * epi.W;
+        orow = (static_cast<int64_t>(img) * (epi.H + 2) + y + 1) * (epi.W + 2) + x + 1;
+      } else if (epi.rowmap == CB_ROWMAP_UNPAD) {
+        const int wp = epi.W + 2, hp = epi.H + 2;
+        const int img = m / (hp * wp);
+        const int r = m - img * (hp * wp);
+        const int y = r / wp, x = r - y * wp;
+        row_ok = row_ok && y >= 1 && y <= epi.H && x >= 1 && x <= epi.W;
+        orow = (static_cast<int64_t>(img) * epi.H + (y - 1)) * epi.W + (x - 1);
+      }
+      orow_half[h] = row_ok ? static_cast<int>(orow) : -1;
     }
 #pragma unroll
     for (int sc = 0; sc < BN / 32; ++sc) {
-      __syncwarp();
-#pragma unroll
-      for (int jj = 0; jj < 4; ++jj) {
-        const int j = sc * 4 + jj;
-        float* p = stg + (lane >> 2) * STG_PITCH + jj * 8 + 2 * (lane & 3);
-        *reinterpret_cast<float2*>(p) = make_float2(acc[4 * j], acc[4 * j + 1]);
-        *reinterpret_cast<float2*>(p + 8 * STG_PITCH) = make_float2(acc[4 * j + 2], acc[4 * j + 3]);
-      }
-      __syncwarp();
-      const int nb = t.n0 + sc * 32 + eh * 16;
-      if (!row_ok || nb >= N) continue;
-      constexpr int NC = 16;
-      float f[NC];
-      const uint32_t srow = smem_u32(stg + er * STG_PITCH + eh * 16);
-#pragma unroll
-      for (int j = 0; j < NC / 4; ++j) {
-        const uint4 u = lds128(srow + j * 16);
-        f[4 * j] = __uint_as_float(u.x); f[4 * j + 1] = __uint_as_float(u.y);
-        f[4 * j + 2] = __uint_as_float(u.z); f[4 * j + 3] = __uint_as_float(u.w);
-      }
-      uint32_t res16[NC / 2], aux16[NC / 2];
-      const int tc = sc * 32 + eh * 16;
-      const int q = (tc & 63) >> 3;
-      if (has_res) {
-#pragma unroll
-        for (int j = 0; j < 2; ++j) {
-          const uint4 u = lds128(swz128(in_buf + (tc >> 6) * IN_BOX_BYTES, wrow + er, q + j));
-          res16[4 * j] = u.x; res16[4 * j + 1] = u.y; res16[4 * j + 2] = u.z; res16[4 * j + 3] = u.w;
-        }
-      }
-      if (has_aux) {
-#pragma unroll
-        for (int j = 0; j < 2; ++j) {
-          const uint4 u = lds128(swz128(in_buf + (has_res ? IN_TILE_BYTES : 0) + (tc >> 6) * IN_BOX_BYTES, wrow + er, q + j));
-          aux16[4 * j] = u.x; aux16[4 * j + 1] = u.y; aux16[4 * j + 2] = u.z; aux16[4 * j + 3] = u.w;
-        }
-      }
-      float shv[NC];
-      if (has_shift) {
-#pragma unroll
-        for (int j = 0; j < NC; j += 4) {
-          float4 s4 = make_float4(0.f, 0.f, 0.f, 0.f);
-          if (nb + j + 4 <= N) s4 = __ldg(reinterpret_cast<const float4*>(epi.shift + nb + j));
-          shv[j] = s4.x; shv[j + 1] = s4.y; shv[j + 2] = s4.z; shv[j + 3] = s4.w;
-        }
-      }
-      uint32_t o2_16[NC / 2];
-      switch (kind) {
-        case EK_SHIFT_ACT: epilogue_shift_act<NC>(f, shv, has_shift, res16, has_res, kind_relu); break;
-        case EK_RELU_MASK: epilogue_relu_mask<NC>(f, res16, has_res, aux16); break;
-        case EK_DROP_RES:
-          epilogue_drop_res<NC>(f, shv, has_shift, res16, has_res, dseed, static_cast<uint64_t>(orow) * static_cast<uint64_t>(N) + nb, epi.drop_thresh,
-                                epi.drop_inv_keep);
-          break;
-        case EK_GELU_STASH: epilogue_gelu_stash<NC>(f, shv, has_shift, o2_16); break;
-        case EK_AUX_MUL: epilogue_aux_mul<NC>(f, res16, has_res, aux16); break;
-        default:
-          if (guard) epilogue_math<NC, true>(f, epi, shv, has_shift, dseed, nb, N, orow, res16, has_res, aux16, has_aux, o2_16, has_out2);
-          else epilogue_math<NC, false>(f, epi, shv, has_shift, dseed, nb, N, orow, res16, has_res, aux16, has_aux, o2_16, has_out2);
-      }
-      if (epi.out_fp32) {
-        float* o = reinterpret_cast<float*>(epi.out) + orow * epi.out_ld + nb;
-#pragma unroll
-        for (int j = 0; j < NC; j += 4)
-          if (nb + j + 4 <= N) *reinterpret_cast<float4*>(o + j) = make_float4(f[j], f[j + 1], f[j + 2], f[j + 3]);
-      } else {
-        __nv_bfloat16* o = reinterpret_cast<__nv_bfloat16*>(epi.out) + orow * epi.out_ld + nb;
-#pragma unroll
-        for (int j = 0; j < 2; ++j)
-          if (nb + 8 * j + 8 <= N)
-            *reinterpret_cast<uint4*>(o + 8 * j) = make_uint4(pack_bf16x2(f[8 * j], f[8 * j + 1]), pack_bf16x2(f[8 * j + 2], f[8 * j + 3]),
-                                                              pack_bf16x2(f[8 * j + 4], f[8 * j + 5]), pack_bf16x2(f[8 * j + 6], f[8 * j + 7]));
-      }
-      if (has_out2) {
-        __nv_bfloat16* o = epi.out2 + orow * epi.out2_ld + nb;
-#pragma unroll
-        for (int j = 0; j < 2; ++j)
-          if (nb + 8 * j + 8 <= N) *reinterpret_cast<uint4*>(o + 8 * j) = make_uint4(o2_16[4 * j], o2_16[4 * j + 1], o2_16[4 * j + 2], o2_16[4 * j + 3]);
+#pragma unroll 1
+      for (int h = 0; h < 2; ++h) {
+        const int wrow = h * 64 + wq * 16;
+        __syncwarp();
+#pragma unroll
+        for (int jj = 0; jj < 4; ++jj) {
+          const int j = sc * 4 + jj;
+          float* p = stg + (lane >> 2) * STG_PITCH + jj * 8 + 2 * (lane & 3);
+          const bool h1 = h != 0;
+          *reinterpret_cast<float2*>(p) = make_float2(h1 ? acc[1][4 * j] : acc[0][4 * j], h1 ? acc[1][4 * j + 1] : acc[0][4 * j + 1]);
+          *reinterpret_cast<float2*>(p + 8 * STG_PITCH) =
+              make_float2(h1 ? acc[1][4 * j + 2] : acc[0][4 * j + 2], h1 ? acc[1][4 * j + 3] : acc[0][4 * j + 3]);
+        }
+        __syncwarp();
+        const int nb = t.n0 + sc * 32 + eh * 16;
+        const int64_t orow = h ? orow_half[1] : orow_half[0];
+        if (orow < 0 || nb >= N) continue;
+        constexpr int NC = 16;
+        float f[NC];
+        const uint32_t srow = smem_u32(stg + er * STG_PITCH + eh * 16);
+#pragma unroll
+        for (int j = 0; j < NC / 4; ++j) {
+          const uint4 u = lds128(srow + j * 16);
+          f[4 * j] = __uint_as_float(u.x); f[4 * j + 1] = __uint_as_float(u.y);
+          f[4 * j + 2] = __uint_as_float(u.z); f[4 * j + 3] = __uint_as_float(u.w);
+        }
+        uint32_t res16[NC / 2], aux16[NC / 2];
+        const int tc = sc * 32 + eh * 16;
+        const int q = (tc & 63) >> 3;
+        if (has_res) {
+#pragma unroll
+          for (int j = 0; j < 2; ++j) {
+            const uint4 u = lds128(swz128(in_buf + (tc >> 6) * IN_BOX_BYTES, wrow + er, q + j));
+            res16[4 * j] = u.x; res16[4 * j + 1] = u.y; res16[4 * j + 2] = u.z; res16[4 * j + 3] = u.w;
+          }
+        }
+        if (has_aux) {
+#pragma unroll
+          for (int j = 0; j < 2; ++j) {
+            const uint4 u = lds128(swz128(in_buf + (has_res ? IN_TILE_BYTES : 0) + (tc >> 6) * IN_BOX_BYTES, wrow + er, q + j));
+            aux16[4 * j] = u.x; aux16[4 * j + 1] = u.y; aux16[4 * j + 2] = u.z; aux16[4 * j + 3] = u.w;
+          }
+        }
+        float shv[NC];
+        if (has_shift) {
+#pragma unroll
+          for (int j = 0; j < NC; j += 4) {
+            float4 s4 = make_float4(0.f, 0.f, 0.f, 0.f);
+            if (nb + j + 4 <= N) s4 = __ldg(reinterpret_cast<const float4*>(epi.shift + nb + j));
+            shv[j] = s4.x; shv[j + 1] = s4.y; shv[j + 2] = s4.z; shv[j + 3] = s4.w;
+          }
+        }
+        uint32_t o2_16[NC / 2];
+        switch (kind) {
+          case EK_SHIFT_ACT: epilogue_shift_act<NC>(f, shv, has_shift, res16, has_res, kind_relu); break;
+          case EK_RELU_MASK: epilogue_relu_mask<NC>(f, res16, has_res, aux16); break;
+          case EK_DROP_RES:
+            epilogue_drop_res<NC>(f, shv, has_shift, res16, has_res, dseed, static_cast<uint64_t>(orow) * static_cast<uint64_t>(N) + nb,
+                                  epi.drop_thresh, epi.drop_inv_keep);
+            break;
+          case EK_GELU_STASH: epilogue_gelu_stash<NC>(f, shv, has_shift, o2_16); break;
+          case EK_AUX_MUL: epilogue_aux_mul<NC>(f, res16, has_res, aux16); break;
+          default:
+            if (guard) epilogue_math<NC, true>(f, epi, shv, has_shift, dseed, nb, N, orow, res16, has_res, aux16, has_aux, o2_16, has_out2);
+            else epilogue_math<NC, false>(f, epi, shv, has_shift, dseed, nb, N, orow, res16, has_res, aux16, has_aux, o2_16, has_out2);
+        }
+        if (epi.out_fp32) {
+          float* o = reinterpret_cast<float*>(epi.out) + orow * epi.out_ld + nb;
+#pragma unroll
+          for (int j = 0; j < NC; j += 4)
+            if (nb + j + 4 <= N) *reinterpret_cast<float4*>(o + j) = make_float4(f[j], f[j + 1], f[j + 2], f[j + 3]);
+        } else {
+          __nv_bfloat16* o = reinterpret_cast<__nv_bfloat16*>(epi.out) + orow * epi.out_ld + nb;
+#pragma unroll
+          for (int j = 0; j < 2; ++j)
+            if (nb + 8 * j + 8 <= N)
+              *reinterpret_cast<uint4*>(o + 8 * j) = make_uint4(pack_bf16x2(f[8 * j], f[8 * j + 1]), pack_bf16x2(f[8 * j + 2], f[8 * j + 3]),
+                                                                pack_bf16x2(f[8 * j + 4], f[8 * j + 5]), pack_bf16x2(f[8 * j + 6], f[8 * j + 7]));
+        }
+        if (has_out2) {
+          __nv_bfloat16* o = epi.out2 + orow * epi.out2_ld + nb;
+#pragma unroll
+          for (int j = 0; j < 2; ++j)
+            if (nb + 8 * j + 8 <= N) *reinterpret_cast<uint4*>(o + 8 * j) = make_uint4(o2_16[4 * j], o2_16[4 * j + 1], o2_16[4 * j + 2], o2_16[4 * j + 3]);
+        }
       }
     }
     if (in_bytes) {
       __syncwarp();
-      if (lane == 0) mbar_arrive(N_IN ? &in_empty[ib] : &empty_bar[s]);
+      if (lane == 0) mbar_arrive(N_IN ? &in_empty[N_IN == 2 ? wg : 0] : &empty_bar[s]);
       if (!N_IN && ++s == STAGES) { s = 0; ph ^= 1; }
     }
+    ring_skip(tile_stages);
+  }
+  if (threadIdx.x == 4 * 32) dbg_stamp(epi, 11);
+}
+
+template <int BN, int OCC>
+__global__ void __launch_bounds__(GEMM_THREADS, OCC)
+    gemm_kernel(const __grid_constant__ CUtensorMap tmA, const __grid_constant__ CUtensorMap tmB, int M, int N, int K, int ntaps, int tap_w,
+                int tap_sign, int iters_per_split, int tiles_m, int tiles_n, int total_tiles, int STAGES, int KCH, GemmEpi epi) {
+  using Cfg = GemmCfg<BN>;
+  extern __shared__ uint8_t smem_raw[];
+  uint8_t* smem = reinterpret_cast<uint8_t*>((reinterpret_cast<uintptr_t>(smem_raw) + 1023) & ~static_cast<uintptr_t>(1023));
+  const int stage_bytes = KCH * Cfg::STAGE_BYTES;
+  uint64_t* full_bar = reinterpret_cast<uint64_t*>(smem + STAGES * stage_bytes);
+  uint64_t* empty_bar = full_bar + MAX_STAGES;
+
+  const int warp = threadIdx.x >> 5;
+  const int lane = threadIdx.x & 31;
+  const int unit = blockIdx.x;
+  const int n_units = gridDim.x;
+  if (threadIdx.x == 0) dbg_stamp(epi, 0);
+  pdl_trigger();
+  if (threadIdx.x == 0) {
+    tma_prefetch_desc(&tmA);
+    tma_prefetch_desc(&tmB);
+    for (int s = 0; s < STAGES; ++s) {
+      mbar_init(&full_bar[s], 1);
+      mbar_init(&empty_bar[s], CONSUMER_WARPS);
+    }
+    fence_mbar_init();
+  }
+  __syncthreads();
+  pdl_wait();
+  if (threadIdx.x == 0) dbg_stamp(epi, 1);
+
+  if (warp >= CONSUMER_WARPS) {
+    if (warp == CONSUMER_WARPS && lane == 0) {
+      int s = 0;
+      uint32_t ph = 0;
+      for (int tile = unit; tile < total_tiles; tile += n_units) {
+        const TileInfo t = decode_tile<BN, 1>(tile, tiles_m, tiles_n, K, ntaps, iters_per_split);
+        int shift = 0;
+        if (ntaps == 9) shift = tap_sign * ((t.tap / 3 - 1) * tap_w + (t.tap % 3 - 1));
+        for (int i = 0; i < t.n_iters; i += KCH) {
+          const int nch = min(KCH, t.n_iters - i);
+          mbar_wait(&empty_bar[s], ph ^ 1);
+          mbar_expect_tx(&full_bar[s], nch * Cfg::STAGE_BYTES);
+          int kit = t.it_begin + i;
+          for (int ch = 0; ch < nch; ++ch, ++kit) {
+            uint8_t* sa = smem + s * stage_bytes + ch * Cfg::STAGE_BYTES;
+            uint8_t* sb = sa + Cfg::A_BYTES;
+            const int p = kit * BK;
+            if (epi.mn3d) {
+              tma_load_3d(sa, &tmA, &full_bar[s], 0, p, t.m0 >> 6);
+              tma_load_3d(sb, &tmB, &full_bar[s], 0, p + shift, t.nb0 >> 6);
+            } else {
+#pragma unroll
+              for (int j = 0; j < BM / 64; ++j) tma_load_2d(sa + j * (BK * 128), &tmA, &full_bar[s], t.m0 + j * 64, p);
+#pragma unroll
+              for (int j = 0; j < BN / 64; ++j) tma_load_2d(sb + j * (BK * 128), &tmB, &full_bar[s], t.nb0 + j * 64, p + shift);
+            }
+          }
+          if (++s == STAGES) { s = 0; ph ^= 1; }
+          if (i == 0 && tile == unit) dbg_stamp(epi, 2);
+        }
+      }
+      dbg_stamp(epi, 3);
+    }
+    return;
+  }
+
+  const int wg = warp >> 2;
+  const int wrow = wg * 64 + (warp & 3) * 16;
+  const uint32_t smem0 = smem_u32(smem);
+  float acc[BN / 2];
+  int s = 0;
+  uint32_t ph = 0;
+  int local = 0;
+  for (int tile = unit; tile < total_tiles; tile += n_units, ++local) {
+    const TileInfo t = decode_tile<BN, 1>(tile, tiles_m, tiles_n, K, ntaps, iters_per_split);
+    if (local == 0 && warp == 0 && lane == 0) dbg_stamp(epi, 4);
+    mma_tile<BN, 1, 1>(acc, smem0, stage_bytes, KCH, STAGES, t.n_iters, wg, lane, s, ph, full_bar, empty_bar);
+    if (local == 0 && warp == 0 && lane == 0) dbg_stamp(epi, 5);
+    wgrad_epilogue<BN>(acc, reinterpret_cast<float*>(epi.out) + static_cast<int64_t>(t.tap) * N, epi.out_ld, epi.scale, M, N,
+                       t.m0 + wrow + (lane >> 2), t.n0, lane);
     if (local == 0 && warp == 0 && lane == 0) dbg_stamp(epi, 8);
   }
   if (threadIdx.x == 0) dbg_stamp(epi, 11);
@@ -605,6 +743,7 @@
 static long long* g_gemm_timeline = nullptr;
 static int g_force_kch = 0;
 static int g_mn3d = 1;
+
 
 struct SmemPlan {
   int epi_bytes, kch, stages, chunk_bytes, n_in;
@@ -626,7 +765,8 @@
   p.stages = chunks_fit / p.kch;
   if (p.stages > MAX_STAGES) p.stages = MAX_STAGES;
   const int stage_iters = ceil_div(kiters, p.kch);
-  if (p.stages > stage_iters + 1) p.stages = stage_iters + 1 > 2 ? stage_iters + 1 : 2;
+  const int cap = staging ? 2 * stage_iters + 1 : (stage_iters + 1 > 2 ? stage_iters + 1 : 2);
+  if (p.stages > cap) p.stages = cap;
   return p;
 }
 static SmemPlan plan_smem(int bn, bool staging, int kiters, int force_kch = 0, int occ = 1, int in_bytes = 0) {
@@ -643,11 +783,15 @@
 
 template <int BN, int MODE, int OCC = 1>
 static int launch_gemm(const cb_gemm_desc& d, const GemmEpi& epi_in, cudaStream_t stream) {
+  static_assert(MODE == 1 || (OCC == 1 && BN <= 128), "TN / NN: one CTA per SM, 128 x 64 or 128 x 128 tiles");
   GemmEpi epi = epi_in;
   using Cfg = GemmCfg<BN>;
   constexpr int LIMIT = OCC == 2 ? SMEM_LIMIT_OCC2 : SMEM_LIMIT;
   static bool attr_set = false;
-  auto kern = gemm_kernel<BN, MODE, OCC>;
+  auto kern = [] {
+    if constexpr (MODE == 1) return gemm_kernel<BN, OCC>;
+    else return gemm_pingpong_kernel<BN, MODE>;
+  }();
   if (!attr_set) {
     cudaError_t e = cudaFuncSetAttribute(kern, cudaFuncAttributeMaxDynamicSharedMemorySize, LIMIT);
     if (e == cudaSuccess && OCC == 2)
@@ -697,15 +841,19 @@
   const int grid = total < units ? total : units;
   const int in_bytes = epi_in_bytes(d, BN);
   const SmemPlan sp = plan_smem(BN, MODE != 1, kiters, (d.reserved >> 8) & 15, OCC, in_bytes);
-  const int epi_bytes = sp.epi_bytes, kch = sp.kch, stages = sp.stages;
+  const int kch = sp.kch, stages = sp.stages;
   if (stages < 2) {
-    set_error("cb_gemm: not enough shared memory for a 2-stage pipeline (BN=%d, epilogue %d B + inputs %d B, %d CTA(s) per SM)", BN, epi_bytes,
-              in_bytes, OCC);
+    set_error("cb_gemm: not enough shared memory for a 2-stage pipeline (BN=%d, epilogue %d B + inputs %d B, %d CTA(s) per SM)", BN,
+              sp.epi_bytes, in_bytes, OCC);
     return CB_ERR_INVALID;
   }
-  const int smem_bytes = stages * kch * Cfg::STAGE_BYTES + sp.n_in * in_bytes + epi_bytes + Cfg::BAR_BYTES + 1024;
-  launch_gemm_k(kern, grid, GEMM_THREADS, smem_bytes, stream, ta, tb, tr, tx, d.m, d.n, d.k, d.ntaps, d.tap_w, d.tap_sign, iters_per_split,
-                tiles_m, tiles_n, total, stages, kch, sp.n_in, epi_bytes, epi);
+  const int smem_bytes = stages * kch * Cfg::STAGE_BYTES + sp.n_in * in_bytes + sp.epi_bytes + Cfg::BAR_BYTES + 1024;
+  if constexpr (MODE == 1)
+    launch_gemm_k(kern, grid, GEMM_THREADS, smem_bytes, stream, ta, tb, d.m, d.n, d.k, d.ntaps, d.tap_w, d.tap_sign, iters_per_split,
+                  tiles_m, tiles_n, total, stages, kch, epi);
+  else
+    launch_gemm_k(kern, grid, PP_THREADS, smem_bytes, stream, ta, tb, tr, tx, d.m, d.n, d.k, d.ntaps, d.tap_w, d.tap_sign, tiles_m,
+                  tiles_n, total, stages, kch, sp.n_in, epi);
   return check_launch("cb_gemm");
 }
 
@@ -720,14 +868,15 @@
   const int units = sm_count() * occ;
   const int kc = ceil_div(d.k, BK);
   const bool wgrad = d.mode == CB_GEMM_WGRAD;
+  const int block_n = (!wgrad && d.block_n == 256) ? 128 : d.block_n;
   static const int cand[3] = {64, 128, 256};
   LaunchCfg best = {0, 1};
   double best_cost = 1e30;
   for (int c = 0; c < 3; ++c) {
     const int bn = cand[c];
     if (occ == 2 && bn > 64) continue;
-    if (d.block_n && bn != d.block_n) continue;
-    if (!d.block_n && !wgrad && bn == 256) continue;
+    if (block_n && bn != block_n) continue;
+    if (!wgrad && bn == 256) continue;
     if (bn > 64 && d.n <= bn / 2) continue;
     const int64_t base = static_cast<int64_t>(ceil_div(d.m, BM)) * ceil_div(d.n, bn) * (wgrad ? d.ntaps : 1);
     const int max_split = wgrad ? (d.split_k > 0 ? d.split_k : (kc < 32 ? kc : 32)) : 1;
@@ -740,8 +889,15 @@
       if (pl.stages < 2) continue;
       const double shallow = (pl.stages * pl.kch < 3 && ips > 2) ? 3.0 : 1.0;
       const double stage_cost = 450.0 + pl.kch * pl.chunk_bytes / (60.0 / occ);
-      const double epi = wgrad ? bn * 24.0 : bn * 30.0;
-      const double cost = rounds * (ceil_div(ips, pl.kch) * stage_cost * shallow + epi) + 2500.0;
+      const double main_loop = ceil_div(ips, pl.kch) * stage_cost * shallow;
+      double cost;
+      if (wgrad) {
+        cost = rounds * (main_loop + bn * 24.0) + 2500.0;
+      } else {
+        const double epi = bn * 30.0;
+        const double per_tile = main_loop > 0.5 * (main_loop + epi) ? main_loop : 0.5 * (main_loop + epi);
+        cost = rounds * per_tile + 0.5 * epi + 2500.0;
+      }
       if (cost < best_cost) {
         best_cost = cost;
         best = {bn, real_sp};
@@ -983,16 +1139,13 @@
     CB_REQUIRE(!(d.out2 && d.out_fp32), "cb_gemm(TN): out2 requires a bf16 primary output");
     CB_REQUIRE(d.rowmap == CB_ROWMAP_NONE || (d.map_h > 0 && d.map_w > 0), "cb_gemm: rowmap needs map_h/map_w");
     CB_REQUIRE(d.ntaps == 1 || d.tap_w > 2, "cb_gemm: tap modes need tap_w (padded row pitch in pixels)");
-    if (want_occ2) {
-      const LaunchCfg l2 = choose_config(d, 2);
-      if (l2.bn == 64) return nn ? launch_gemm<64, 2, 2>(d, epi, stream) : launch_gemm<64, 0, 2>(d, epi, stream);
-    }
+    CB_REQUIRE(d.block_n == 0 || d.block_n == 64 || d.block_n == 128 || d.block_n == 256, "cb_gemm: block_n must be 0, 64, 128 or 256 (got %d)",
+               d.block_n);
     const LaunchCfg lc = choose_config(d);
     switch (lc.bn) {
       case 64: return nn ? launch_gemm<64, 2>(d, epi, stream) : launch_gemm<64, 0>(d, epi, stream);
       case 128: return nn ? launch_gemm<128, 2>(d, epi, stream) : launch_gemm<128, 0>(d, epi, stream);
-      case 256: return nn ? launch_gemm<256, 2>(d, epi, stream) : launch_gemm<256, 0>(d, epi, stream);
-      default: CB_REQUIRE(false, "cb_gemm: block_n must be 0, 64, 128 or 256 (got %d)", lc.bn);
+      default: CB_REQUIRE(false, "cb_gemm: no tile width for block_n %d", d.block_n);
     }
   } else {
     CB_REQUIRE(d.out_fp32 == 1, "cb_gemm(WGRAD): output must be fp32");
```
